# schwallergroup/matinvent

Hardware: AMD Instinct MI355X
Metric: crystal structures/sec (1000-step reverse diffusion) (higher is better)
Workload: dtype f32 via 2-plane fp16 split (3 fp16 MFMA terms, f32 accumulate)

## Files before the change

matinvent_amd/csrc/backward.hip:

```cpp
#include "gemm_split.h"
#include "net.h"

namespace mi {
extern int g_edge_pairs;
int g_tn_xsilu = 1;
int g_bwd_pairs_tile = 1;
int g_bwd_pairs_fused = 1;
int g_bwd_dz2_planes = 1;
int g_bwd_wgrad_planes = 1;
int g_bwd_head_window = 1;
int g_bwd_wgrad_f16 = 1;
}

namespace mi {

__global__ void transpose_kernel(const float* __restrict__ src, int ld_src, int rows, int cols, float* __restrict__ dst) {
    int idx = blockIdx.x * blockDim.x + threadIdx.x;
    if (idx >= rows * cols) return;
    int c = idx / rows, r = idx % rows;
    dst[idx] = src[(size_t)r * ld_src + c];
}

__global__ void silu_bwd_kernel(const float* __restrict__ dy, const float* __restrict__ z, float* __restrict__ out, int64_t n) {
    int64_t i = (int64_t)blockIdx.x * blockDim.x + threadIdx.x;
// ... 1221 lines not shown
    const float s2 = sigma * sigma;
#pragma unroll
    for (int i = -10; i <= 10; ++i) {
        float v = x + (float)i;
        float e = expf(-(v * v) / 2.0f / s2);
        num += v / s2 * e;
        den += e;
    }
    return num / den;
}

struct NoiseArgs {
    const float *lengths, *angles, *frac0;
    const int* atom_types;
    const float *rand_l, *rand_x, *rand_t;
    const int* node_off;
    float *in_lat, *in_frac, *in_types, *tar_x;
    float *out_rand_l, *out_rand_t;
    float c0, c1, sigma, sigma_norm;
    uint64_t seed;
    uint32_t step;
    int64_t node_offset, graph_offset;
    int stack_B0 = 0, stack_N0 = 0;
    float sc0[MI_MAX_STACK], sc1[MI_MAX_STACK], ssig[MI_MAX_STACK], ssn[MI_MAX_STACK];
    const float* sched = nullptr;
};

__global__ __launch_bounds__(256) void add_noise_kernel(NoiseArgs a) {
    const int b = blockIdx.x, tid = threadIdx.x;
    const int cp = a.stack_B0 ? b / a.stack_B0 : 0;
    const float c0 = a.sched ? a.sched[b * 4] : a.stack_B0 ? a.sc0[cp] : a.c0, c1 = a.sched ? a.sched[b * 4 + 1] : a.stack_B0 ? a.sc1[cp] : a.c1;
    const float sigma = a.sched ? a.sched[b * 4 + 2] : a.stack_B0 ? a.ssig[cp] : a.sigma;
    const float sigma_norm = a.sched ? a.sched[b * 4 + 3] : a.stack_B0 ? a.ssn[cp] : a.sigma_norm;
    const uint32_t step = a.step + (uint32_t)cp;
    const int64_t gsub = (int64_t)cp * a.stack_B0, nsub = (int64_t)cp * a.stack_N0;
    __shared__ float Lm[9];
    if (tid == 0) lattice_matrix(a.lengths + b * 3, a.angles + b * 3, Lm);
    __syncthreads();
    if (tid < 9) {
        int idx = b * 9 + tid;
        float z = a.rand_l ? a.rand_l[idx] : philox_normal1(a.seed, step, DRAW_FT_L, (uint64_t)(a.graph_offset - gsub) * 9 + idx);
        a.out_rand_l[idx] = z;
        a.in_lat[idx] = c0 * Lm[tid] + c1 * z;
    }
    const int n0 = a.node_off[b], n1 = a.node_off[b + 1];
    for (int idx = n0 * 3 + tid; idx < n1 * 3; idx += 256) {
        float z = a.rand_x ? a.rand_x[idx] : philox_normal1(a.seed, step, DRAW_FT_X, (uint64_t)(a.node_offset - nsub) * 3 + idx);
        float sx = sigma * z;
        a.in_frac[idx] = pymod1(a.frac0[idx] + sx);
        a.tar_x[idx] = d_log_p_wn(sx, sigma) / sqrtf(sigma_norm);
    }
    for (int64_t idx = (int64_t)n0 * MI_NUM_TYPES + tid; idx < (int64_t)n1 * MI_NUM_TYPES; idx += 256) {
        int i = (int)(idx / MI_NUM_TYPES), k = (int)(idx % MI_NUM_TYPES);
        float z = a.rand_t ? a.rand_t[idx] : philox_normal1(a.seed, step, DRAW_FT_T, (uint64_t)(a.node_offset - nsub) * MI_NUM_TYPES + idx);
        float onehot = (a.atom_types[i] - 1 == k) ? 1.f : 0.f;
        a.out_rand_t[idx] = z;
        a.in_types[idx] = c0 * onehot + c1 * z;
    }
}

struct StackTimes {
    int t[MI_MAX_STACK];
};
__global__ void fill_stack_times_kernel(int* __restrict__ times, StackTimes st, int B0, int B) {
    int b = blockIdx.x * blockDim.x + threadIdx.x;
    if (b < B) times[b] = st.t[b / B0];
}


}

using namespace mi;

extern "C" {

int mi_cspnet_forward_train(mi_net* net, mi_batch* b, const float* t_emb, const float* atom_types, const float* frac,
                            const float* lattices, float* lattice_out, float* coord_out, float* type_out, void* stream) {
    MI_POOL_STREAM(b, stream, "mi_cspnet_forward_train");
    MI_CHECK(net && b, MI_EINVAL, "null handle");
    MI_CHECK(b->H == net->H && b->L == net->L, MI_EINVAL, "batch was created for a different network");
    MI_TRY(net_tape_prepare(net, b));
    return net_forward(net, b, t_emb, atom_types, frac, lattices, lattice_out, coord_out, type_out, (hipStream_t)stream, true);
}

int mi_cspnet_backward(mi_net* net, mi_batch* b, const float* d_lattice_out, const float* d_coord_out, const float* d_type_out,
                       float* grad_theta, void* stream) {
    MI_POOL_STREAM(b, stream, "mi_cspnet_backward");
    MI_CHECK(net && b && d_lattice_out && d_coord_out && d_type_out && grad_theta, MI_EINVAL, "null argument");
    MI_CHECK(net->W2T != nullptr, MI_ESTATE, "mi_net_set_params must run before backward");
    return net_backward(net, b, d_lattice_out, d_coord_out, d_type_out, grad_theta, (hipStream_t)stream);
}

int mi_batch_set_wgrad_window(mi_net* net, mi_batch* b, int micro_steps) {
    MI_CHECK(net && b, MI_EINVAL, "null handle");
    MI_CHECK(b->H == net->H && b->L == net->L, MI_EINVAL, "batch was created for a different network");
    return net_wgrad_window(net, b, micro_steps);
}

int mi_cspnet_wgrad_flush(mi_net* net, mi_batch* b, float* grad_theta, void* stream) {
    MI_POOL_STREAM(b, stream, "mi_cspnet_wgrad_flush");
    MI_CHECK(net && b && grad_theta, MI_EINVAL, "null argument");
    return net_wgrad_flush(net, b, grad_theta, (hipStream_t)stream);
}

int mi_batch_wgrad_pending(const mi_batch* b) { return b ? b->tape.wcur : 0; }

int mi_adam_step(float* theta, const float* grad, float* exp_avg, float* exp_avg_sq, int64_t n, int step, float lr, float beta1,
                 float beta2, float eps, float grad_scale, void* stream) {
    MI_CHECK(theta && grad && exp_avg && exp_avg_sq && n >= 0 && step >= 1, MI_EINVAL, "bad argument");
    if (n == 0) return MI_OK;
    const double bc1 = 1.0 - pow((double)beta1, step), bc2 = 1.0 - pow((double)beta2, step);
    hipLaunchKernelGGL(adam_kernel, dim3((unsigned)cdiv(n, 256)), dim3(256), 0, (hipStream_t)stream, theta, grad, exp_avg, exp_avg_sq, n,
                       (float)(lr / bc1), (float)(1.0 / sqrt(bc2)), beta1, beta2, eps, grad_scale);
    MI_KERNEL_CHECK();
    return MI_OK;
}

int mi_add_noise(mi_batch* b, const float* lengths, const float* angles, const float* frac0, const int* atom_types, float c0, float c1,
                 float sigma, float sigma_norm, uint64_t seed, uint32_t step, const float* rand_l, const float* rand_x, const float* rand_t,
                 float* in_lattice, float* in_frac, float* in_types, float* tar_x, float* out_rand_l, float* out_rand_t, void* stream) {
    MI_NO_POOLED(b, "mi_add_noise");
    MI_CHECK(b && lengths && angles && frac0 && atom_types && in_lattice && in_frac && in_types && tar_x && out_rand_l && out_rand_t,
             MI_EINVAL, "null argument");
    if (b->B == 0) return MI_OK;
    NoiseArgs a{lengths, angles, frac0, atom_types, rand_l, rand_x, rand_t, b->node_off, in_lattice, in_frac, in_types, tar_x,
                out_rand_l, out_rand_t, c0, c1, sigma, sigma_norm, seed, step, b->node_offset, b->graph_offset};
    hipLaunchKernelGGL(add_noise_kernel, dim3(b->B), dim3(256), 0, (hipStream_t)stream, a);
    MI_KERNEL_CHECK();
    return MI_OK;
}

int mi_add_noise_per_crystal(mi_batch* b, const float* lengths, const float* angles, const float* frac0, const int* atom_types,
                             const float* sched, uint64_t seed, uint32_t step, const float* rand_l, const float* rand_x, const float* rand_t,
                             float* in_lattice, float* in_frac, float* in_types, float* tar_x, float* out_rand_l, float* out_rand_t,
                             void* stream) {
    MI_CHECK(b && lengths && angles && frac0 && atom_types && sched && in_lattice && in_frac && in_types && tar_x && out_rand_l && out_rand_t,
             MI_EINVAL, "null argument");
    if (b->B == 0) return MI_OK;
    NoiseArgs a{lengths, angles, frac0, atom_types, rand_l, rand_x, rand_t, b->node_off, in_lattice, in_frac, in_types, tar_x,
                out_rand_l, out_rand_t, 0.f, 0.f, 0.f, 0.f, seed, step, b->node_offset, b->graph_offset};
    a.sched = sched;
    hipLaunchKernelGGL(add_noise_kernel, dim3(b->B), dim3(256), 0, (hipStream_t)stream, a);
    MI_KERNEL_CHECK();
    return MI_OK;
}

}

namespace mi {

int ft_micro_run(const char* what, mi_net* agent, mi_batch* ab, mi_net* prior, mi_batch* pb, const float* lengths, const float* angles,
                 const float* frac0, const int* atom_types, const float* time_freqs, int t, float c0, float c1, float sigma_t, float sigma_norm,
                 int copies, const int* ts, const float* c0s, const float* c1s, const float* sigmas, const float* sigma_norms, uint64_t seed,
                 uint32_t noise_step, const float* rand_l, const float* rand_x, const float* rand_t, float cost_lattice, float cost_coord,
                 float cost_type, int accum_steps, float* grad_theta, ft_loss_stage_fn stage, void* stage_ctx, void* stream, void* aux_stream) {
    MI_CHECK(agent && ab && prior && pb && lengths && angles && frac0 && atom_types && time_freqs && grad_theta && stage, MI_EINVAL,
             "null argument");
    TraceRange range(what);
    MI_CHECK(ab != pb, MI_EINVAL, "agent and prior need separate batch handles (separate workspace)");
    MI_CHECK(ab->B == pb->B && ab->N == pb->N && accum_steps >= 1, MI_EINVAL, "inconsistent batch arguments");
    hipStream_t s = (hipStream_t)stream;
    const int B = ab->B, N = ab->N;
    if (B == 0 || N == 0) return MI_OK;
    MI_TRY(net_tape_prepare(agent, ab));
    Tape& tp = ab->tape;
    const bool hw = tp.head_window();
    const size_t hs = hw ? (size_t)tp.wcur : 0;
    float* const nz_types = hw ? tp.w_types + hs * N * MI_NUM_TYPES : tp.nz_types;
    float* const temb = hw ? tp.w_temb + hs * B * agent->TD : ab->temb;
    float* const d_t = hw ? tp.w_dtype + hs * N * MI_NUM_TYPES : tp.d_t;
    float* const d_x = hw ? tp.w_dcoord + hs * N * 3 : tp.d_x;
    NoiseArgs na{lengths, angles, frac0, atom_types, rand_l, rand_x, rand_t, ab->node_off, tp.nz_lat, tp.nz_frac, nz_types, tp.tar_x,
                 tp.rnd_l, tp.rnd_t, c0, c1, sigma_t, sigma_norm, seed, noise_step, ab->node_offset, ab->graph_offset};
    if (copies > 0) {
        MI_CHECK(copies <= MI_MAX_STACK && B % copies == 0 && N % copies == 0 && ts && c0s && c1s && sigmas && sigma_norms, MI_EINVAL,
                 "stacked micro-step: %d replicas do not fit the batch (B = %d, N = %d) or the limit %d", copies, B, N, MI_MAX_STACK);
        StackTimes st;
        na.stack_B0 = B / copies;
        na.stack_N0 = N / copies;
        for (int c = 0; c < copies; ++c) {
            st.t[c] = ts[c];
            na.sc0[c] = c0s[c];
            na.sc1[c] = c1s[c];
            na.ssig[c] = sigmas[c];
            na.ssn[c] = sigma_norms[c];
        }
        hipLaunchKernelGGL(fill_stack_times_kernel, dim3(cdiv(B, 256)), dim3(256), 0, s, ab->times, st, na.stack_B0, B);
    } else {
        hipLaunchKernelGGL(fill_int_kernel2, dim3(cdiv(B, 256)), dim3(256), 0, s, ab->times, t, B);
    }
    MI_TRY(mi_time_embedding(ab->times, time_freqs, B, agent->TD, temb, stream));
    hipLaunchKernelGGL(add_noise_kernel, dim3(B), dim3(256), 0, s, na);
    MI_KERNEL_CHECK();
    if (aux_stream && aux_stream != stream) {
        hipStream_t s2 = (hipStream_t)aux_stream;
        if (!pb->ev_fork) {
            MI_HIP(hipEventCreateWithFlags(&pb->ev_fork, hipEventDisableTiming));
            MI_HIP(hipEventCreateWithFlags(&pb->ev_join, hipEventDisableTiming));
        }
        MI_HIP(hipEventRecord(pb->ev_fork, s));
        MI_HIP(hipStreamWaitEvent(s2, pb->ev_fork, 0));
        MI_TRY(net_forward(prior, pb, temb, nz_types, tp.nz_frac, tp.nz_lat, pb->pred_l, pb->pred_x, pb->pred_t, s2, false));
        MI_HIP(hipEventRecord(pb->ev_join, s2));
        tp.borrow_inputs = true;
        const int rc = net_forward(agent, ab, temb, nz_types, tp.nz_frac, tp.nz_lat, ab->pred_l, ab->pred_x, ab->pred_t, s, true);
        tp.borrow_inputs = false;
        MI_TRY(rc);
        MI_HIP(hipStreamWaitEvent(s, pb->ev_join, 0));
    } else {
        tp.borrow_inputs = true;
        const int rc = net_forward(agent, ab, temb, nz_types, tp.nz_frac, tp.nz_lat, ab->pred_l, ab->pred_x, ab->pred_t, s, true);
        tp.borrow_inputs = false;
        MI_TRY(rc);
        MI_TRY(net_forward(prior, pb, temb, nz_types, tp.nz_frac, tp.nz_lat, pb->pred_l, pb->pred_x, pb->pred_t, s, false));
    }
    FtStageIO io{ab->pred_l, ab->pred_x, ab->pred_t, pb->pred_l, pb->pred_x, pb->pred_t, tp.rnd_l, tp.tar_x, tp.rnd_t, ab->node_off,
                 tp.d_l, d_x, d_t, tp.Lb, tp.KLb, B, N, cost_lattice, cost_coord, cost_type, accum_steps};
    MI_TRY(stage(io, stage_ctx, s));
    return net_backward(agent, ab, tp.d_l, d_x, d_t, grad_theta, s);
}

}

struct FtRewardStage {
    const float* reward;
    float kl_sigma;
    int b_global;
    float *stats, *out_sample_loss, *out_kl;
};
static int ft_reward_stage(const FtStageIO& io, void* ctx, hipStream_t s) {
    const FtRewardStage& c = *(const FtRewardStage*)ctx;
    const int B = io.B;
    LossArgs la{io.pl, io.px, io.pt, io.plp, io.pxp, io.ptp, io.rl, io.tx, io.rt, c.reward, io.node_off,
                io.dl, io.dx, io.dt, io.Lb, io.KLb, io.cl, io.cx, io.ct, c.kl_sigma,
                1.0f / ((float)c.b_global * (float)io.accum_steps)};
    hipLaunchKernelGGL(ft_loss_kernel, dim3(B), dim3(256), 0, s, la);
    if (c.stats) hipLaunchKernelGGL(ft_stats_kernel, dim3(1), dim3(64), 0, s, io.Lb, io.KLb, c.reward, B, c.kl_sigma, 1.0f / (float)c.b_global, c.stats);
    MI_KERNEL_CHECK();
    if (c.out_sample_loss) MI_HIP(hipMemcpyAsync(c.out_sample_loss, io.Lb, B * 4, hipMemcpyDeviceToDevice, s));
    if (c.out_kl) MI_HIP(hipMemcpyAsync(c.out_kl, io.KLb, B * 4, hipMemcpyDeviceToDevice, s));
    return MI_OK;
}

static int ft_micro_impl(mi_net* agent, mi_batch* ab, mi_net* prior, mi_batch* pb, const float* lengths, const float* angles,
                         const float* frac0, const int* atom_types, const float* reward, const float* time_freqs, int t, float c0, float c1,
                         float sigma_t, float sigma_norm, int copies, const int* ts, const float* c0s, const float* c1s, const float* sigmas,
                         const float* sigma_norms, uint64_t seed, uint32_t noise_step, const float* rand_l, const float* rand_x,
                         const float* rand_t, float cost_lattice, float cost_coord, float cost_type, float kl_sigma, int b_global,
                         int accum_steps, float* grad_theta, float* stats, float* out_sample_loss, float* out_kl, void* stream,
                         void* aux_stream) {
    MI_CHECK(reward, MI_EINVAL, "null argument");
    MI_CHECK(!ab || b_global >= ab->B / (copies > 0 ? copies : 1), MI_EINVAL, "inconsistent batch arguments");
    FtRewardStage st{reward, kl_sigma, b_global, stats, out_sample_loss, out_kl};
    return ft_micro_run("mi_ft_micro_step", agent, ab, prior, pb, lengths, angles, frac0, atom_types, time_freqs, t, c0, c1, sigma_t, sigma_norm,
                        copies, ts, c0s, c1s, sigmas, sigma_norms, seed, noise_step, rand_l, rand_x, rand_t, cost_lattice, cost_coord, cost_type,
                        accum_steps, grad_theta, ft_reward_stage, &st, stream, aux_stream);
}

extern "C" {

int mi_ft_micro_step(mi_net* agent, mi_batch* ab, mi_net* prior, mi_batch* pb, const float* lengths, const float* angles,
                     const float* frac0, const int* atom_types, const float* reward, const float* time_freqs, int t, float c0, float c1,
                     float sigma_t, float sigma_norm, uint64_t seed, uint32_t noise_step, const float* rand_l, const float* rand_x,
                     const float* rand_t, float cost_lattice, float cost_coord, float cost_type, float kl_sigma, int b_global, int accum_steps,
                     float* grad_theta, float* stats, float* out_sample_loss, float* out_kl, void* stream, void* aux_stream) {
    MI_NO_LATENT(agent, "mi_ft_micro_step");
    MI_NO_LATENT(prior, "mi_ft_micro_step");
    MI_NO_POOLED(ab, "mi_ft_micro_step");
    MI_NO_POOLED(pb, "mi_ft_micro_step");
    return ft_micro_impl(agent, ab, prior, pb, lengths, angles, frac0, atom_types, reward, time_freqs, t, c0, c1, sigma_t, sigma_norm, 0, nullptr,
                         nullptr, nullptr, nullptr, nullptr, seed, noise_step, rand_l, rand_x, rand_t, cost_lattice, cost_coord, cost_type,
                         kl_sigma, b_global, accum_steps, grad_theta, stats, out_sample_loss, out_kl, stream, aux_stream);
}

int mi_ft_micro_steps_stacked(mi_net* agent, mi_batch* ab, mi_net* prior, mi_batch* pb, const float* lengths, const float* angles,
                              const float* frac0, const int* atom_types, const float* reward, const float* time_freqs, int copies,
                              const int* t_host, const float* c0_host, const float* c1_host, const float* sigma_t_host,
                              const float* sigma_norm_host, uint64_t seed, uint32_t noise_step, const float* rand_l, const float* rand_x,
                              const float* rand_t, float cost_lattice, float cost_coord, float cost_type, float kl_sigma, int b_global,
                              int accum_steps, float* grad_theta, float* stats, void* stream, void* aux_stream) {
    MI_NO_LATENT(agent, "mi_ft_micro_steps_stacked");
    MI_NO_LATENT(prior, "mi_ft_micro_steps_stacked");
    MI_NO_POOLED(ab, "mi_ft_micro_steps_stacked");
    MI_NO_POOLED(pb, "mi_ft_micro_steps_stacked");
    MI_CHECK(copies >= 1, MI_EINVAL, "copies must be positive");
    return ft_micro_impl(agent, ab, prior, pb, lengths, angles, frac0, atom_types, reward, time_freqs, 0, 0.f, 0.f, 0.f, 0.f, copies, t_host,
                         c0_host, c1_host, sigma_t_host, sigma_norm_host, seed, noise_step, rand_l, rand_x, rand_t, cost_lattice, cost_coord,
                         cost_type, kl_sigma, b_global, accum_steps, grad_theta, stats, nullptr, nullptr, stream, aux_stream);
}

int mi_debug_gemm(int kind, const float* A, int lda, const float* W, int ldw, float* C, int ldc, int M, int N, int K, void* stream) {
    MI_CHECK(A && W && C, MI_EINVAL, "null argument");
    if (kind == 2 || kind == 3) {
        static u16 *pa = nullptr, *pw = nullptr;
        static size_t na = 0, nw = 0;
        hipStream_t s = (hipStream_t)stream;
        if (planes_elems(M, K) > na) { if (pa) (void)hipFree(pa); na = planes_elems(M, K); MI_HIP(hipMalloc((void**)&pa, na * 2)); }
        if (planes_elems(N, K) > nw) { if (pw) (void)hipFree(pw); nw = planes_elems(N, K); MI_HIP(hipMalloc((void**)&pw, nw * 2)); }
        Planes PA = make_planes(pa, K, PL_S_LN), PW = make_planes(pw, K, PL_SW);
        if (ldc >= 0) {
            hipLaunchKernelGGL(split_planes_kernel<>, dim3(cdiv((int64_t)((M + 127) / 128 * 128) * PA.KT * 16, 256)), dim3(256), 0, s, A, lda, M, K, PA);
            hipLaunchKernelGGL(split_planes_kernel<>, dim3(cdiv((int64_t)((N + 127) / 128 * 128) * PW.KT * 16, 256)), dim3(256), 0, s, W, ldw, N, K, PW);
        }
        if (MI_PLANES_FP16 && (N & 255) == 0 && (K & 63) == 0 && K >= 128) {
            static u16* pf = nullptr;
            static size_t nf = 0;
            if (frag_elems(N, K) > nf) { if (pf) (void)hipFree(pf); nf = frag_elems(N, K); MI_HIP(hipMalloc((void**)&pf, nf * 2)); }
            MI_TRY(pack_frag_from_planes(PW, N, K, pf, s));
            PW.frag = pf;
        }
        PlanesEpilogue pe;
        pe.C = C;
        pe.ldc = ldc < 0 ? -ldc : ldc;
        const int saved = g_planes_variant;
        g_planes_variant = kind == 3;
        const int rc = gemm_planes(PA, PW, M, N, K, pe, s);
        g_planes_variant = saved;
        return rc;
    }
#if MI_PLANES_FP16
    if (kind == 5) {
        hipStream_t s = (hipStream_t)stream;
        MI_CHECK(M % 256 == 0 && N % 128 == 0 && K >= 4096, MI_EINVAL, "kind 5: the plane-set weight-gradient form needs M % 256 == 0, N % 128 == 0, K >= 4096");
        static u16 *pa = nullptr, *pw = nullptr;
        static float *sc = nullptr, *dsc = nullptr;
        static size_t na = 0, nw = 0;
        const size_t ea = planes_elems(K, M), ew = planes_elems(K, N), scf = (size_t)1 << 25;
        if (ea > na) { if (pa) (void)hipFree(pa); na = ea; MI_HIP(hipMalloc((void**)&pa, na * 2)); }
        if (ew > nw) { if (pw) (void)hipFree(pw); nw = ew; MI_HIP(hipMalloc((void**)&pw, nw * 2)); }
        if (!sc) MI_HIP(hipMalloc((void**)&sc, scf * sizeof(float)));
        if (!dsc) {
            MI_HIP(hipMalloc((void**)&dsc, 2 * sizeof(float)));
            const float h[2] = {64.f, 1.f / 64.f};
            MI_HIP(hipMemcpy(dsc, h, sizeof(h), hipMemcpyHostToDevice));
        }
        Planes PA = make_planes(pa, M, 64.f), PW = make_planes(pw, N, 64.f);
        hipLaunchKernelGGL(split_planes_kernel<>, dim3(cdiv((int64_t)((K + 127) / 128 * 128) * PA.KT * 16, 256)), dim3(256), 0, s, A, lda, K, M, PA);
        hipLaunchKernelGGL(split_planes_kernel<>, dim3(cdiv((int64_t)((K + 127) / 128 * 128) * PW.KT * 16, 256)), dim3(256), 0, s, W, ldw, K, N, PW);
        MI_KERNEL_CHECK();
        MI_CHECK(gemm_tn_planes_ok(PA, 0, PW, 0, K, M, N), MI_EINVAL, "kind 5: shape outside the plane-set form");
        return gemm_tn_planes(PA, 0, PW, 0, C, ldc, K, M, N, dsc, dsc, sc, scf, s);
    }
#endif
    if (kind == 4) {
        static float* sc = nullptr;
        const size_t scf = (size_t)1 << 24;
        if (!sc) MI_HIP(hipMalloc((void**)&sc, scf * sizeof(float)));
        return gemm_tn_auto(A, lda, W, ldw, C, ldc, K, M, N, sc, scf, (hipStream_t)stream);
    }
    return kind == 0 ? gemm_nt_f32(A, lda, W, ldw, C, ldc, M, N, K, GemmEpilogue(), (hipStream_t)stream)
                     : gemm_nt_split(A, lda, W, ldw, C, ldc, M, N, K, GemmEpilogue(), (hipStream_t)stream);
}

}
```

matinvent_amd/csrc/edge_stage.hip:

```cpp
#include <mutex>

#include <cstdio>
#include <cstdlib>
#include "net.h"
#include "gemm_split.h"
#define MI_LOOP_BARRIER() __builtin_amdgcn_s_barrier()
#define MI_RING_WAIT(w) asm volatile("s_waitcnt vmcnt(20)" : "+v"((w)[0][0]), "+v"((w)[0][1]), "+v"((w)[1][0]), "+v"((w)[1][1]))

namespace mi {

extern int g_edge2_train;
int g_edge2_fused = 1;

#if MI_PLANES_FP16

struct EdgeGemm2Args {
    Planes A;
    const u16* W2f;
    const float* b2;
    const float* dsc;
    const int* src;
    const int* rowptr;
    float* part;
    int E, N;
    const int* tab = nullptr;
    float* Z2 = nullptr;
    unsigned long long* clk;
};

constexpr int EG2_TAB = 2 + 128 + 128;
__global__ __launch_bounds__(128) void edge2_tables_kernel(const int* __restrict__ src, const int* __restrict__ rowptr, int E, int N, int* __restrict__ tab) {
    const int tile = blockIdx.x, tid = threadIdx.x, row0 = tile * 128;
    if (row0 >= E) return;
    const int nrows = E - row0 < 128 ? E - row0 : 128;
    const int node_first = src[row0];
    int* t = tab + (size_t)tile * EG2_TAB;
    const int r = row0 + tid, node = node_first + tid;
    t[2 + tid] = r < E ? src[r] - node_first : -1;
    t[130 + tid] = node < N ? tile - (rowptr[node] >> 7) : 0;
    if (tid == 0) {
        t[0] = node_first;
        t[1] = src[row0 + nrows - 1] - node_first + 1;
    }
}

constexpr int EG2B_STAGE = 2 * 128 * 64, EG2B_NST = 4;
constexpr int EG2B_LDS = EG2B_NST * EG2B_STAGE + 128 * 4 + 128 * 4;

template <int D, bool SAVE_Z = false>
__global__ __launch_bounds__(256) __attribute__((amdgpu_waves_per_eu(2, 2))) void edge_gemm2b_kernel(EdgeGemm2Args a) {
    constexpr int H = 512, KS = H / 16, KT = H / 32;
    extern __shared__ __attribute__((aligned(16))) unsigned char smem[];
    int* srcl = reinterpret_cast<int*>(smem + EG2B_NST * EG2B_STAGE);
    int* slotb = srcl + 128;
    const int tid = threadIdx.x, lane = tid & 63, wave = __builtin_amdgcn_readfirstlane(tid >> 6);
    const int l31 = lane & 31, kg = lane >> 5;
    const int id = blockIdx.x, slot = id >> 3, half = slot & 1, tile = (slot >> 1) * 8 + (id & 7);
    const int row0 = tile * 128;
    if (row0 >= a.E) return;
    const int nrows = a.E - row0 < 128 ? a.E - row0 : 128;
    int stamp_i = 0;
    auto stamp = [&]() {
        if (a.clk && tid == 0) a.clk[(size_t)(tile * 2 + half) * 8 + stamp_i] = __builtin_amdgcn_s_memtime();
        ++stamp_i;
    };
    stamp();
    if (a.clk && tid == 0) a.clk[(size_t)(tile * 2 + half) * 8 + 4] = __builtin_amdgcn_s_memrealtime();

    const int* tab = a.tab + (size_t)tile * EG2_TAB;
    int t_srcl = -1, t_slotb = 0;
    if (tid < 128) {
        t_srcl = tab[2 + tid];
        t_slotb = tab[130 + tid];
    }
    const int node_first = tab[0], cnt_tab = tab[1];

    const __amdgpu_buffer_rsrc_t rsa = uniform_rsrc(a.A.base + a.A.tile(tile, 0), a.A.KT * 24576);
    const int voffa = (lane >> 2) * 64 + (((lane & 3) ^ ((lane >> 4) & 3)) << 4);
    auto dma_tile = [&](int kt, int st) {
#pragma unroll
        for (int q = 0; q < 4; ++q) {
            const int piece = wave * 4 + q;
            __builtin_amdgcn_raw_ptr_buffer_load_lds(rsa, (__attribute__((address_space(3))) void*)(smem + st * EG2B_STAGE + piece * 1024), 16, voffa,
                                                     kt * 24576 + (piece >> 3) * 8192 + (piece & 7) * 1024, 0, 0);
        }
    };
    dma_tile(0, 0);
    dma_tile(1, 1);
    dma_tile(2, 2);

    int voffw[2];
#pragma unroll
    for (int t = 0; t < 2; ++t) voffw[t] = lane * 16 + ((8 * half + 2 * wave + t) * KS) * 2048;
    u32x4 ring[D][2][2];
    const u32x4 rsw_s = rsrc_words(a.W2f, H * H * 4);
    auto ring_load = [&](int ks, u32x4 (&w)[2][2]) {
        const int soff = __builtin_amdgcn_readfirstlane(ks * 2048);
#pragma unroll
        for (int t = 0; t < 2; ++t) {
            asm volatile("buffer_load_dwordx4 %0, %1, %2, %3 offen" : "=v"(w[t][0]) : "v"(voffw[t]), "s"(rsw_s), "s"(soff));
            asm volatile("buffer_load_dwordx4 %0, %1, %2, %3 offen offset:1024" : "=v"(w[t][1]) : "v"(voffw[t]), "s"(rsw_s), "s"(soff));
        }
    };
#pragma unroll
    for (int d = 0; d < D; ++d) ring_load(d, ring[d]);

    if (tid < 128) {
        srcl[tid] = t_srcl;
        slotb[tid] = t_slotb;
    }
    const float os = a.dsc[1] * (1.f / PL_SW), s_m2 = a.dsc[2], inv_m2 = a.dsc[3];

    f32x16 acc[4][2];
#pragma unroll
    for (int i = 0; i < 4; ++i)
#pragma unroll
        for (int j = 0; j < 2; ++j)
#pragma unroll
            for (int r = 0; r < 16; ++r) acc[i][j][r] = 0.f;
    const unsigned lds0 = (unsigned)(uintptr_t)(__attribute__((address_space(3))) unsigned char*)smem;
    unsigned rd_off[2];
#pragma unroll
    for (int s2 = 0; s2 < 2; ++s2) rd_off[s2] = lds0 + (unsigned)(l31 * 64 + (((2 * s2 + kg) ^ ((l31 >> 2) & 3)) * 16));
    auto read_a = [&](int st, int s2, f16x8 (&af)[4][2]) {
        const unsigned va = rd_off[s2] + (unsigned)st * EG2B_STAGE;
#define MI_RD128(dst, off) asm volatile("ds_read_b128 %0, %1 offset:%2" : "=v"(dst) : "v"(va), "n"(off))
        MI_RD128(af[0][0], 0 * 2048);        MI_RD128(af[0][1], 0 * 2048 + 8192);
        MI_RD128(af[1][0], 1 * 2048);        MI_RD128(af[1][1], 1 * 2048 + 8192);
        MI_RD128(af[2][0], 2 * 2048);        MI_RD128(af[2][1], 2 * 2048 + 8192);
        MI_RD128(af[3][0], 3 * 2048);        MI_RD128(af[3][1], 3 * 2048 + 8192);
#undef MI_RD128
    };
    auto mma = [&](const u32x4 (&w)[2][2], f16x8 (&af)[4][2]) {
#pragma unroll
        for (int ip = 0; ip < 2; ++ip) {
            if (ip == 0) asm volatile("s_waitcnt lgkmcnt(4)" : "+v"(af[0][0]), "+v"(af[0][1]), "+v"(af[1][0]), "+v"(af[1][1]));
            else asm volatile("s_waitcnt lgkmcnt(0)" : "+v"(af[2][0]), "+v"(af[2][1]), "+v"(af[3][0]), "+v"(af[3][1]));
#pragma unroll
            for (int term = MI_TERM0; term < 3; ++term)
#pragma unroll
                for (int i = 2 * ip; i < 2 * ip + 2; ++i)
#pragma unroll
                    for (int j = 0; j < 2; ++j)
                        acc[i][j] = __builtin_amdgcn_mfma_f32_32x32x16_f16(af[i][term == 0 ? 1 : 0], __builtin_bit_cast(f16x8, w[j][term == 1 ? 1 : 0]), acc[i][j], 0, 0, 0);
        }
    };
    static_assert(D == 4, "two k-tiles of ring per unrolled pair of iterations");
#pragma unroll 1
    for (int kt = 0; kt < KT; kt += 2) {
#pragma unroll
        for (int h2 = 0; h2 < 2; ++h2) {
            const int k = kt + h2;
            if (k == 0 || k >= KT - 3) asm volatile("s_waitcnt vmcnt(0)" ::: "memory");
            else asm volatile("s_waitcnt vmcnt(24)" ::: "memory");
            MI_LOOP_BARRIER();
            if (k == 0) stamp();
            if (k + 3 < KT) dma_tile(k + 3, (k + 3) & 3);
            f16x8 af[4][2];
#pragma unroll
            for (int s2 = 0; s2 < 2; ++s2) {
                read_a(k & 3, s2, af);
                MI_RING_WAIT(ring[2 * h2 + s2]);
                mma(ring[2 * h2 + s2], af);
                if (2 * k + s2 + D < KS) ring_load(2 * k + s2 + D, ring[2 * h2 + s2]);
                __builtin_amdgcn_sched_barrier(0);
            }
        }
    }
    stamp();

    if constexpr (SAVE_Z) {
        __syncthreads();
        float* stage = reinterpret_cast<float*>(smem) + wave * 1152;
#pragma unroll
        for (int i = 0; i < 4; ++i)
#pragma unroll
            for (int j = 0; j < 2; ++j) {
                const int rb = row0 + i * 32, cb = half * 256 + wave * 64 + j * 32;
#pragma unroll
                for (int r = 0; r < 16; ++r) stage[((r & 3) + 8 * (r >> 2) + 4 * kg) * 36 + l31] = acc[i][j][r] * os;
                __builtin_amdgcn_wave_barrier();
#pragma unroll
                for (int u = 0; u < 2; ++u) {
                    const int q = lane + 64 * u, rl = q >> 2, c8 = (q & 3) * 8;
                    const int row = rb + rl, col = cb + c8;
                    f32x4 z0 = *reinterpret_cast<const f32x4*>(stage + rl * 36 + c8);
                    f32x4 z1 = *reinterpret_cast<const f32x4*>(stage + rl * 36 + c8 + 4);
                    if (row < a.E) {
                        z0 += *reinterpret_cast<const f32x4*>(a.b2 + col);
                        z1 += *reinterpret_cast<const f32x4*>(a.b2 + col + 4);
                        float* d = a.Z2 + (size_t)row * H + col;
                        *reinterpret_cast<f32x4*>(d) = z0;
                        *reinterpret_cast<f32x4*>(d + 4) = z1;
                    }
                }
                __builtin_amdgcn_wave_barrier();
            }
    }

    const int cnt = nrows > 0 ? cnt_tab : 0;
    u16* sfr = reinterpret_cast<u16*>(smem);
    unsigned sat = 0;
    const int nlb = (cnt + 31) >> 5;
    __syncthreads();
    for (int f = tid; f < nlb * 8 * 64; f += 256) {
        const int ln = f & 63, fu = (f >> 6) & 1, frb = (f >> 7) & 3, fq = f >> 9;
        const int me = fq * 32 + (ln & 31), fkg = ln >> 5;
        u32x4 w;
#pragma unroll
        for (int i2 = 0; i2 < 4; ++i2) {
            const int ia = 2 * i2, ib = 2 * i2 + 1;
            const int ra = frb * 32 + 4 * fkg + 8 * (2 * fu + (ia >> 2)) + (ia & 3), rbb = frb * 32 + 4 * fkg + 8 * (2 * fu + (ib >> 2)) + (ib & 3);
            w[i2] = (srcl[ra] == me ? 0x3C00u : 0u) | (srcl[rbb] == me ? 0x3C000000u : 0u);
        }
        *reinterpret_cast<u32x4*>(sfr + (size_t)f * 8) = w;
    }
    __syncthreads();
#pragma unroll
    for (int j = 0; j < 2; ++j) {
        __builtin_amdgcn_sched_barrier(0);
        const int col = half * 256 + wave * 64 + j * 32 + l31;
        const float bcol = a.b2[col];
#pragma unroll 1
        for (int lb0 = 0; lb0 < nlb; lb0 += 2) {
            const bool two = lb0 + 1 < nlb;
            f32x16 ps[2];
#pragma unroll
            for (int q = 0; q < 2; ++q)
#pragma unroll
                for (int r = 0; r < 16; ++r) ps[q][r] = 0.f;
#pragma unroll
            for (int rb = 0; rb < 4; ++rb) {
                const f32x16 av = acc[rb][j];
#pragma unroll
                for (int u = 0; u < 2; ++u) {
                    f16x8 mh, ml;
#pragma unroll
                    for (int idx = 0; idx < 8; idx += 2) {
                        const float v0 = silu_fast(av[8 * u + idx] * os + bcol), v1 = silu_fast(av[8 * u + idx + 1] * os + bcol);
                        unsigned p[3];
                        pl_split_pair_acc(v0, v1, s_m2, p, sat);
                        const f16x2 h = __builtin_bit_cast(f16x2, p[0]), lo = __builtin_bit_cast(f16x2, p[1]);
                        mh[idx] = h[0]; mh[idx + 1] = h[1];
                        ml[idx] = lo[0]; ml[idx + 1] = lo[1];
                    }
#pragma unroll
                    for (int q = 0; q < 2; ++q) {
                        if (q == 1 && !two) break;
                        const f16x8 sf = *reinterpret_cast<const f16x8*>(sfr + (size_t)((((lb0 + q) * 4 + rb) * 2 + u) * 64 + lane) * 8);
                        ps[q] = __builtin_amdgcn_mfma_f32_32x32x16_f16(sf, ml, ps[q], 0, 0, 0);
                        ps[q] = __builtin_amdgcn_mfma_f32_32x32x16_f16(sf, mh, ps[q], 0, 0, 0);
                    }
                    __builtin_amdgcn_sched_barrier(0);
                }
            }
#pragma unroll
            for (int q = 0; q < 2; ++q)
#pragma unroll
                for (int r = 0; r < 16; ++r) {
                    const int loc = (lb0 + q) * 32 + (r & 3) + 8 * (r >> 2) + 4 * kg;
                    if (loc < cnt) a.part[((size_t)slotb[loc] * a.N + node_first + loc) * H + col] = ps[q][r] * inv_m2;
                }
        }
    }
    stamp();
    if (a.clk && tid == 0) a.clk[(size_t)(tile * 2 + half) * 8 + 5] = __builtin_amdgcn_s_memrealtime();
    sat_report(sat);
}

template <bool EXT, bool LEAN = false>
__global__ __launch_bounds__(256) __attribute__((amdgpu_waves_per_eu(2, 2))) void gemm_rt_kernel(Planes A, const u16* __restrict__ Wf, int M, int N, int K,
                                                                                                 PlanesEpilogue pe, unsigned long long* __restrict__ clk) {
    const int KS = K >> 4, KT = K >> 5;
    extern __shared__ __attribute__((aligned(16))) unsigned char smem[];
    M = pe.rows(M);
    const int tid = threadIdx.x, lane = tid & 63, wave = __builtin_amdgcn_readfirstlane(tid >> 6);
    int stamp_i = 0;
    auto stamp = [&]() {
        if (clk && tid == 0) clk[(size_t)blockIdx.x * 8 + stamp_i] = __builtin_amdgcn_s_memtime();
        ++stamp_i;
    };
    stamp();
    if (clk && tid == 0) clk[(size_t)blockIdx.x * 8 + 4] = __builtin_amdgcn_s_memrealtime();
    const int l31 = lane & 31, kg = lane >> 5;
    const int ncb = N >> 8;
    const int id = blockIdx.x, slot = id >> 3, cb = slot % ncb, tile = (slot / ncb) * 8 + (id & 7);
    const int row0 = tile * 128;
    if (row0 >= M) return;

    const __amdgpu_buffer_rsrc_t rsa = uniform_rsrc(A.base + A.tile(tile, 0), A.KT * 24576);
    const int voffa = (lane >> 2) * 64 + (((lane & 3) ^ ((lane >> 4) & 3)) << 4);
    auto dma_tile = [&](int kt, int st) {
#pragma unroll
        for (int q = 0; q < 4; ++q) {
            const int piece = wave * 4 + q;
            __builtin_amdgcn_raw_ptr_buffer_load_lds(rsa, (__attribute__((address_space(3))) void*)(smem + st * EG2B_STAGE + piece * 1024), 16, voffa,
                                                     kt * 24576 + (piece >> 3) * 8192 + (piece & 7) * 1024, 0, 0);
        }
    };
    dma_tile(0, 0);
    dma_tile(1, 1);
    dma_tile(2, 2);

    int voffw[2];
#pragma unroll
    for (int t = 0; t < 2; ++t) voffw[t] = lane * 16 + ((8 * cb + 2 * wave + t) * KS) * 2048;
    u32x4 ring[4][2][2];
    const u32x4 rsw_s = rsrc_words(Wf, N * K * 4);
    auto ring_load = [&](int ks, u32x4 (&w)[2][2]) {
        const int soff = __builtin_amdgcn_readfirstlane(ks * 2048);
#pragma unroll
        for (int t = 0; t < 2; ++t) {
            asm volatile("buffer_load_dwordx4 %0, %1, %2, %3 offen" : "=v"(w[t][0]) : "v"(voffw[t]), "s"(rsw_s), "s"(soff));
            asm volatile("buffer_load_dwordx4 %0, %1, %2, %3 offen offset:1024" : "=v"(w[t][1]) : "v"(voffw[t]), "s"(rsw_s), "s"(soff));
        }
    };
#pragma unroll
    for (int d = 0; d < 4; ++d) ring_load(d, ring[d]);

    f32x16 acc[4][2];
#pragma unroll
    for (int i = 0; i < 4; ++i)
#pragma unroll
        for (int j = 0; j < 2; ++j)
#pragma unroll
            for (int r = 0; r < 16; ++r) acc[i][j][r] = 0.f;
    const unsigned lds0 = (unsigned)(uintptr_t)(__attribute__((address_space(3))) unsigned char*)smem;
    unsigned rd_off[2];
#pragma unroll
    for (int s2 = 0; s2 < 2; ++s2) rd_off[s2] = lds0 + (unsigned)(l31 * 64 + (((2 * s2 + kg) ^ ((l31 >> 2) & 3)) * 16));
    auto read_a = [&](int st, int s2, f16x8 (&af)[4][2]) {
        const unsigned va = rd_off[s2] + (unsigned)st * EG2B_STAGE;
#define MI_RD128(dst, off) asm volatile("ds_read_b128 %0, %1 offset:%2" : "=v"(dst) : "v"(va), "n"(off))
        MI_RD128(af[0][0], 0 * 2048);        MI_RD128(af[0][1], 0 * 2048 + 8192);
        MI_RD128(af[1][0], 1 * 2048);        MI_RD128(af[1][1], 1 * 2048 + 8192);
        MI_RD128(af[2][0], 2 * 2048);        MI_RD128(af[2][1], 2 * 2048 + 8192);
        MI_RD128(af[3][0], 3 * 2048);        MI_RD128(af[3][1], 3 * 2048 + 8192);
#undef MI_RD128
    };
    auto mma = [&](const u32x4 (&w)[2][2], f16x8 (&af)[4][2]) {
#pragma unroll
        for (int ip = 0; ip < 2; ++ip) {
            if (ip == 0) asm volatile("s_waitcnt lgkmcnt(4)" : "+v"(af[0][0]), "+v"(af[0][1]), "+v"(af[1][0]), "+v"(af[1][1]));
            else asm volatile("s_waitcnt lgkmcnt(0)" : "+v"(af[2][0]), "+v"(af[2][1]), "+v"(af[3][0]), "+v"(af[3][1]));
#pragma unroll
            for (int term = MI_TERM0; term < 3; ++term)
#pragma unroll
                for (int i = 2 * ip; i < 2 * ip + 2; ++i)
#pragma unroll
                    for (int j = 0; j < 2; ++j)
                        if constexpr (LEAN)
                            acc[i][j] = __builtin_amdgcn_mfma_f32_32x32x16_f16(__builtin_bit_cast(f16x8, w[j][term == 1 ? 1 : 0]), af[i][term == 0 ? 1 : 0], acc[i][j], 0, 0, 0);
                        else
                            acc[i][j] = __builtin_amdgcn_mfma_f32_32x32x16_f16(af[i][term == 0 ? 1 : 0], __builtin_bit_cast(f16x8, w[j][term == 1 ? 1 : 0]), acc[i][j], 0, 0, 0);
        }
    };
#pragma unroll 1
    for (int kt = 0; kt < KT; kt += 2) {
#pragma unroll
        for (int h2 = 0; h2 < 2; ++h2) {
            const int k = kt + h2;
            if (k == 0 || k >= KT - 3) asm volatile("s_waitcnt vmcnt(0)" ::: "memory");
            else asm volatile("s_waitcnt vmcnt(24)" ::: "memory");
            MI_LOOP_BARRIER();
            if (k == 0) stamp();
            if (k + 3 < KT) dma_tile(k + 3, (k + 3) & 3);
            f16x8 af[4][2];
#pragma unroll
            for (int s2 = 0; s2 < 2; ++s2) {
                read_a(k & 3, s2, af);
                MI_RING_WAIT(ring[2 * h2 + s2]);
                mma(ring[2 * h2 + s2], af);
                if (2 * k + s2 + 4 < KS) ring_load(2 * k + s2 + 4, ring[2 * h2 + s2]);
                __builtin_amdgcn_sched_barrier(0);
            }
        }
    }
    __syncthreads();
    stamp();
    if constexpr (LEAN) planes_epilogue_lean<4, 2>(pe, acc, tile, cb * 256 + wave * 64, M, lane);
    else planes_epilogue_rows<4, 2, EXT>(pe, acc, row0, cb * 256 + wave * 64, M, N, lane, reinterpret_cast<float*>(smem) + wave * 1152);
    stamp();
    if (clk && tid == 0) clk[(size_t)blockIdx.x * 8 + 5] = __builtin_amdgcn_s_memrealtime();
}

__global__ void pack_frag_from_planes_kernel(Planes W, int N, int K, u16* __restrict__ dst) {
    const int KS = K / 16;
    const int64_t idx = (int64_t)blockIdx.x * blockDim.x + threadIdx.x;
    if (idx >= (int64_t)N * (K / 8)) return;
    const int r = (int)(idx / (K / 8)), ch = (int)(idx % (K / 8));
    const int ct = r >> 5, l31 = r & 31, ks = ch >> 1, kg = ch & 1;
#pragma unroll
    for (int pl = 0; pl < 2; ++pl)
        *reinterpret_cast<u32x4*>(dst + ((((size_t)ct * KS + ks) * 2 + pl) * 64 + kg * 32 + l31) * 8) = *reinterpret_cast<const u32x4*>(W.base + W.elem(r, ch * 8, pl));
}

int g_edge1_fused = 9;

__global__ void pack_frag_wff_pair_kernel(const float* __restrict__ W1, int edge_in, int H, int F, int Kh, u16* __restrict__ dst) {
    const int K = 2 * Kh, KS = K / 16, F3 = 3 * F;
    const int64_t idx = (int64_t)blockIdx.x * blockDim.x + threadIdx.x;
    if (idx >= (int64_t)H * (K / 8)) return;
    const int r = (int)(idx / (K / 8)), ch = (int)(idx % (K / 8));
    const int ct = r >> 5, l31 = r & 31, ks = ch >> 1, kg = ch & 1;
    float v[8];
#pragma unroll
    for (int i = 0; i < 8; ++i) {
        const int c = ch * 8 + i, blk = c >= Kh, cc = blk ? c - Kh : c;
        v[i] = cc < F3 ? W1[(size_t)r * edge_in + 2 * H + 9 + blk * F3 + cc] : 0.f;
    }
    u32x4 pk[2];
#pragma unroll
    for (int i = 0; i < 4; ++i) {
        unsigned p[3];
        pl_split_pair(v[2 * i], v[2 * i + 1], PL_SW, p);
        pk[0][i] = p[0];
        pk[1][i] = p[1];
    }
#pragma unroll
    for (int pl = 0; pl < 2; ++pl) *reinterpret_cast<u32x4*>(dst + ((((size_t)ct * KS + ks) * 2 + pl) * 64 + kg * 32 + l31) * 8) = pk[pl];
}

template <int D, bool WIDE>
__device__ __forceinline__ void edge_gemm1_body(const Planes& A, const u16* __restrict__ Wf, int M, int N, int K, PlanesEpilogue& pe, unsigned long long* clk) {
    extern __shared__ __attribute__((aligned(16))) unsigned char smem[];
    const int tid = threadIdx.x, lane = tid & 63, wave = __builtin_amdgcn_readfirstlane(tid >> 6);
    const int l31 = lane & 31, kg = lane >> 5;
    constexpr int MI = 4, NJ = 1;
    constexpr int WM = 4 / MI, WN = 4 / WM, WGC = 32 * NJ * WN;
    const int KT = K / 32, KS = K / 16, nq = N / WGC;
    const int wm = wave / WN, wn = wave % WN;
    const int id = blockIdx.x;
    float cps_local = 0.f;
    auto eval_scales = [&]() {
        if (pe.sc_pq) {
            float dsc[6];
            act_scales_eval(__uint_as_float(pe.sc_pq[0]), __uint_as_float(pe.sc_gmax[0]), pe.sc_wb, dsc);
            cps_local = dsc[0];
            if (id == 0 && tid < 6) {
                pe.sc_dsc[tid] = dsc[tid];
                if (pe.sc_dsc2) pe.sc_dsc2[tid] = dsc[tid];
            }
        }
    };
    eval_scales();
    if (pe.diag_C0 && id >= pe.diag_block0) {
        const float cps = cps_local != 0.f ? cps_local : pe.Cp.s();
        const int n0 = (id - pe.diag_block0) * 8, n1 = n0 + 8 < pe.diag_nodes ? n0 + 8 : pe.diag_nodes;
        const float* PQ = pe.ep.row_bias;
        const int ldpq = pe.ep.ld_row_bias;
        for (int f = 2 * tid; f < N; f += 512) {
            const float c0 = pe.diag_C0[f], c1 = pe.diag_C0[f + 1];
            for (int i = n0; i < n1; ++i) {
                const int e = pe.diag_e[i], g = pe.diag_node2graph[i];
                const float* G = pe.ep.row_bias3 + (size_t)g * pe.ep.ld_row_bias3;
                const float v0 = c0 + ((PQ[(size_t)i * ldpq + f] + PQ[(size_t)i * ldpq + N + f]) + G[f]);
                const float v1 = c1 + ((PQ[(size_t)i * ldpq + f + 1] + PQ[(size_t)i * ldpq + N + f + 1]) + G[f + 1]);
                if (pe.ep.pre_act) {
                    pe.ep.pre_act[(size_t)e * pe.ep.ld_pre + f] = v0;
                    pe.ep.pre_act[(size_t)e * pe.ep.ld_pre + f + 1] = v1;
                }
                unsigned p[3];
                pl_split_pair(silu_fast(v0), silu_fast(v1), cps, p);
#pragma unroll
                for (int k = 0; k < NPL; ++k) *reinterpret_cast<unsigned*>(pe.Cp.base + pe.Cp.elem(e, f, k)) = p[k];
            }
        }
        return;
    }
    const int slot = id >> 3, qt = slot % nq, tile = (slot / nq) * 8 + (id & 7);
    const int row0 = tile * 128;
    if (row0 >= M) return;
    int stamp_i = 0;
    auto stamp = [&]() {
        if (clk && tid == 0) clk[(size_t)(tile * nq + qt) * 8 + stamp_i] = __builtin_amdgcn_s_memtime();
        ++stamp_i;
    };
    stamp();

    const __amdgpu_buffer_rsrc_t rsa = uniform_rsrc(A.base + A.tile(tile, 0), A.KT * 24576);
    const int voffa = (lane >> 2) * 64 + (((lane & 3) ^ ((lane >> 4) & 3)) << 4);
    auto dma_tile = [&](int kt, int st) {
#pragma unroll
        for (int q = 0; q < 4; ++q) {
            const int piece = wave * 4 + q;
            __builtin_amdgcn_raw_ptr_buffer_load_lds(rsa, (__attribute__((address_space(3))) void*)(smem + st * EG2B_STAGE + piece * 1024), 16, voffa,
                                                     kt * 24576 + (piece >> 3) * 8192 + (piece & 7) * 1024, 0, 0);
        }
    };
    dma_tile(0, 0);
    dma_tile(1, 1);
    dma_tile(2, 2);
    const __amdgpu_buffer_rsrc_t rsw = uniform_rsrc(Wf, N * K * 4);
    int voffw[NJ];
#pragma unroll
    for (int t = 0; t < NJ; ++t) voffw[t] = lane * 16 + (((WN * qt + wn) * NJ + t) * KS) * 2048;
    u32x4 ring[D][NJ][2];
    const u32x4 rsw_s = rsrc_words(Wf, N * K * 4);
    auto ring_load = [&](int ks, u32x4 (&w)[NJ][2]) {
        const int soff = __builtin_amdgcn_readfirstlane(ks * 2048);
        asm volatile("buffer_load_dwordx4 %0, %1, %2, %3 offen" : "=v"(w[0][0]) : "v"(voffw[0]), "s"(rsw_s), "s"(soff));
        asm volatile("buffer_load_dwordx4 %0, %1, %2, %3 offen offset:1024" : "=v"(w[0][1]) : "v"(voffw[0]), "s"(rsw_s), "s"(soff));
    };
#pragma unroll
    for (int d = 0; d < D; ++d) ring_load(d, ring[d]);

    f32x16 acc[MI][NJ], accS[MI][NJ];
#pragma unroll
    for (int i = 0; i < MI; ++i)
#pragma unroll
        for (int j = 0; j < NJ; ++j)
#pragma unroll
            for (int r = 0; r < 16; ++r) acc[i][j][r] = 0.f;
    const unsigned lds0 = (unsigned)(uintptr_t)(__attribute__((address_space(3))) unsigned char*)smem;
    unsigned rd_off[2];
#pragma unroll
    for (int s2 = 0; s2 < 2; ++s2) rd_off[s2] = lds0 + (unsigned)(l31 * 64 + (((2 * s2 + kg) ^ ((l31 >> 2) & 3)) * 16));
    auto read_a = [&](int st, int s2, f16x8 (&af)[MI][2]) {
        const unsigned va = rd_off[s2] + (unsigned)st * EG2B_STAGE;
#define MI_RD128(dst, off) asm volatile("ds_read_b128 %0, %1 offset:%2" : "=v"(dst) : "v"(va), "n"(off))
        MI_RD128(af[0][0], 0 * 2048);        MI_RD128(af[0][1], 0 * 2048 + 8192);
        MI_RD128(af[1][0], 1 * 2048);        MI_RD128(af[1][1], 1 * 2048 + 8192);
        MI_RD128(af[2][0], 2 * 2048);        MI_RD128(af[2][1], 2 * 2048 + 8192);
        MI_RD128(af[3][0], 3 * 2048);        MI_RD128(af[3][1], 3 * 2048 + 8192);
#undef MI_RD128
    };
    auto mma = [&](u32x4 (&w)[NJ][2], f16x8 (&af)[MI][2]) {
        asm volatile("s_waitcnt vmcnt(14)" : "+v"(w[0][0]), "+v"(w[0][1]));
#pragma unroll
        for (int ip = 0; ip < 2; ++ip) {
            if (ip == 0) asm volatile("s_waitcnt lgkmcnt(4)" : "+v"(af[0][0]), "+v"(af[0][1]), "+v"(af[1][0]), "+v"(af[1][1]));
            else asm volatile("s_waitcnt lgkmcnt(0)" : "+v"(af[2][0]), "+v"(af[2][1]), "+v"(af[3][0]), "+v"(af[3][1]));
#pragma unroll
            for (int term = MI_TERM0; term < 3; ++term)
#pragma unroll
                for (int i = 2 * ip; i < 2 * ip + 2; ++i)
                    acc[i][0] = __builtin_amdgcn_mfma_f32_32x32x16_f16(af[i][term == 0 ? 1 : 0], __builtin_bit_cast(f16x8, w[0][term == 1 ? 1 : 0]), acc[i][0], 0, 0, 0);
        }
    };
    static_assert(D == 4, "two k-tiles of ring per unrolled pair of iterations");
    const int khalf = KT / 2;
#pragma unroll 1
    for (int kt = 0; kt < KT; kt += 2) {
#pragma unroll
        for (int h2 = 0; h2 < 2; ++h2) {
            const int k = kt + h2;
            if (k == khalf) {
#pragma unroll
                for (int i = 0; i < MI; ++i)
#pragma unroll
                    for (int j = 0; j < NJ; ++j) {
                        accS[i][j] = acc[i][j];
#pragma unroll
                        for (int r = 0; r < 16; ++r) acc[i][j][r] = 0.f;
                    }
            }
            if (k == 0 || k >= KT - 3) asm volatile("s_waitcnt vmcnt(0)" ::: "memory");
            else asm volatile("s_waitcnt vmcnt(16)" ::: "memory");
            MI_LOOP_BARRIER();
            if (k == 0) stamp();
            if (k + 3 < KT) dma_tile(k + 3, (k + 3) & 3);
            f16x8 af[MI][2];
#pragma unroll
            for (int s2 = 0; s2 < 2; ++s2) {
                read_a(k & 3, s2, af);
                mma(ring[2 * h2 + s2], af);
                if (2 * k + s2 + D < KS) ring_load(2 * k + s2 + D, ring[2 * h2 + s2]);
                __builtin_amdgcn_sched_barrier(0);
            }
        }
    }
    stamp();
    __syncthreads();
    planes_epilogue_pairs<MI, NJ, WIDE>(pe, accS, acc, row0 + wm * MI * 32, qt * WGC + wn * 32 * NJ, M, N, lane, reinterpret_cast<float*>(smem) + wave * 2304, cps_local);
    stamp();
}

template <int D, bool WIDE = true>
__global__ __launch_bounds__(256) __attribute__((amdgpu_waves_per_eu(2, 2))) void edge_gemm1b_kernel(Planes A, const u16* __restrict__ Wf, int M, int N, int K,
                                                                                                     PlanesEpilogue pe, unsigned long long* clk) {
    edge_gemm1_body<D, WIDE>(A, Wf, M, N, K, pe, clk);
}

unsigned long long* g_edge1_clk = nullptr;

__global__ void empty_boundary_kernel() {}

int edge_gemm1(mi_net* net, const Planes& A, int layer, int M, PlanesEpilogue pe, hipStream_t s) {
    if (g_ablate_skip & 2) return MI_OK;
    if (g_ablate_skip & 32) hipLaunchKernelGGL(empty_boundary_kernel, dim3(1), dim3(64), 0, s);
    static std::once_flag once;
    static hipError_t attr_err = hipSuccess;
    std::call_once(once, [] {
        attr_err = hipFuncSetAttribute((const void*)edge_gemm1b_kernel<4>, hipFuncAttributeMaxDynamicSharedMemorySize, EG2B_LDS);
        if (attr_err == hipSuccess) attr_err = hipFuncSetAttribute((const void*)edge_gemm1b_kernel<4, false>, hipFuncAttributeMaxDynamicSharedMemorySize, EG2B_LDS);
    });
    MI_HIP(attr_err);
    const int H = net->H, K = 2 * net->Kh;
    count_mfma(M, H, K, MI_PLANES_TERMS);
    pe.out_scale = 1.f / (A.scale * PL_SW);
    int nblk = (H / 128) * ((cdiv(M, 128) + 7) / 8 * 8);
    if (pe.diag_C0) {
        pe.diag_block0 = nblk;
        nblk += cdiv(pe.diag_nodes, 8);
    }
    const u16* Wf = net->Wffc + (size_t)layer * ((size_t)H * K * 2);
    if (pe.pair_wide) hipLaunchKernelGGL((edge_gemm1b_kernel<4>), dim3(nblk), dim3(256), EG2B_LDS, s, A, Wf, M, H, K, pe, g_edge1_clk);
    else hipLaunchKernelGGL((edge_gemm1b_kernel<4, false>), dim3(nblk), dim3(256), EG2B_LDS, s, A, Wf, M, H, K, pe, g_edge1_clk);
    MI_KERNEL_CHECK();
    return MI_OK;
}

bool edge_gemm1_supported(const mi_net* net, int64_t M) {
    if (!(net->H % 128 == 0 && net->Wffc != nullptr && (2 * net->Kh) % 64 == 0) || g_edge1_fused == 0) return false;
    if (g_edge1_fused != 9) return true;
    return (int64_t)(net->H / 128) * ((cdiv(M, 128) + 7) / 8 * 8) > g_planes_lat_max_blocks;
}

int edge_gemm1_pack(mi_net* net, int l, const float* W1, hipStream_t s) {
    const int H = net->H, K = 2 * net->Kh;
    hipLaunchKernelGGL(pack_frag_wff_pair_kernel, dim3(cdiv((int64_t)H * (K / 8), 256)), dim3(256), 0, s, W1, net->edge_in, H, net->F, net->Kh,
                       net->Wffc + (size_t)l * ((size_t)H * K * 2));
    MI_KERNEL_CHECK();
    return MI_OK;
}

unsigned long long* g_edge2_clk = nullptr;

int edge_gemm2(mi_net* net, mi_batch* b, int layer, hipStream_t s, float* Z2) {
    if (g_ablate_skip & 4) return MI_OK;
    if (g_ablate_skip & 32) hipLaunchKernelGGL(empty_boundary_kernel, dim3(1), dim3(64), 0, s);
    static std::once_flag once;
    static hipError_t attr_err = hipSuccess;
    std::call_once(once, [] {
        attr_err = hipFuncSetAttribute((const void*)edge_gemm2b_kernel<4>, hipFuncAttributeMaxDynamicSharedMemorySize, EG2B_LDS);
        if (attr_err == hipSuccess) attr_err = hipFuncSetAttribute((const void*)edge_gemm2b_kernel<4, true>, hipFuncAttributeMaxDynamicSharedMemorySize, EG2B_LDS);
    });
    MI_HIP(attr_err);
    const int H = net->H;
    count_mfma(b->E, H, H, MI_PLANES_TERMS);
    EdgeGemm2Args a;
    a.A = make_planes(b->m1_cur ? b->m1_cur : b->M1pl, H, PL_S_ACT, b->dsc);
    a.W2f = net->Wnc + (size_t)layer * node_chain_pack_elems(H) + (size_t)5 * H * H * 2;
    a.b2 = net->p("csp_layer_" + std::to_string(layer) + ".edge_mlp.2.bias");
    a.dsc = b->dsc;
    a.src = b->src;
    a.rowptr = b->rowptr;
    a.part = b->part;
    a.E = (int)b->E;
    a.N = b->N;
    {
        const int tiles_cap = cdiv(b->E_cap, 128);
        if (!b->e2_tab) MI_TRY(dev_alloc(b, &b->e2_tab, (size_t)tiles_cap * EG2_TAB));
        if (b->e2_tab_epoch != b->graph_epoch) {
            hipLaunchKernelGGL(edge2_tables_kernel, dim3(cdiv(b->E, 128)), dim3(128), 0, s, b->src, b->rowptr, (int)b->E, b->N, b->e2_tab);
            MI_KERNEL_CHECK();
            b->e2_tab_epoch = b->graph_epoch;
        }
        a.tab = b->e2_tab;
    }
    a.Z2 = Z2;
    a.clk = g_edge2_clk;
    if (Z2) {
        hipLaunchKernelGGL((edge_gemm2b_kernel<4, true>), dim3(2 * ((cdiv(b->E, 128) + 7) / 8 * 8)), dim3(256), EG2B_LDS, s, a);
        MI_KERNEL_CHECK();
        return MI_OK;
    }
    hipLaunchKernelGGL((edge_gemm2b_kernel<4>), dim3(2 * ((cdiv(b->E, 128) + 7) / 8 * 8)), dim3(256), EG2B_LDS, s, a);
    MI_KERNEL_CHECK();
    return MI_OK;
}

bool edge_gemm2_supported(const mi_net* net) { return g_edge2_fused && net->H == 512 && net->Wnc != nullptr; }

unsigned long long* g_rt_clk = nullptr;
int g_rt_clk_ext = -1;
int g_rt_lean = 1;
int g_rt_clk_skip = 0;

int gemm_rt(const Planes& A, const u16* Wfrag, int M, int N, int K, const PlanesEpilogue& pe, bool ext, hipStream_t s) {
    static std::once_flag once;
    static hipError_t attr_err = hipSuccess;
    std::call_once(once, [] {
        attr_err = hipFuncSetAttribute((const void*)gemm_rt_kernel<false>, hipFuncAttributeMaxDynamicSharedMemorySize, EG2B_NST * EG2B_STAGE);
        if (attr_err == hipSuccess) attr_err = hipFuncSetAttribute((const void*)gemm_rt_kernel<true>, hipFuncAttributeMaxDynamicSharedMemorySize, EG2B_NST * EG2B_STAGE);
        if (attr_err == hipSuccess) attr_err = hipFuncSetAttribute((const void*)gemm_rt_kernel<false, true>, hipFuncAttributeMaxDynamicSharedMemorySize, EG2B_NST * EG2B_STAGE);
        if (const char* e = getenv("MI_RT_LEAN")) g_rt_lean = atoi(e) & 3;
    });
    MI_HIP(attr_err);
    MI_CHECK(Wfrag && (N & 255) == 0 && (K & 63) == 0 && K >= 128 && A.KT >= K / 32, MI_EINVAL, "gemm_rt: N % 256, K % 64, K >= 128 and a fragment-order W operand");
    if (M <= 0) return MI_OK;
    count_mfma(M, N, K, MI_PLANES_TERMS);
    const dim3 grid((N >> 8) * ((cdiv(M, 128) + 7) / 8 * 8));
    static const bool trace = getenv("MI_RT_TRACE") != nullptr;
    if (trace)
        fprintf(stderr, "gemm_rt M=%d N=%d K=%d ext=%d act=%d bias=%d rb=%d%d%d pre_add=%d pre_act=%d res=%d res_pl=%d os=%g res2=%d res2_pl=%d rows2=%d post_mul=%d C=%d Cp=%d absmax=%d\n", M, N, K,
                (int)ext, pe.ep.act, !!pe.ep.bias, !!pe.ep.row_bias, !!pe.ep.row_bias2, !!pe.ep.row_bias3, !!pe.ep.pre_add, !!pe.ep.pre_act, !!pe.ep.residual, !!pe.res_pl.base,
                (double)pe.ep.out_scale, !!pe.residual2, !!pe.res2_pl.base, !!pe.res2_rows, !!pe.post_mul, !!pe.C, !!pe.Cp.base, !!pe.absmax);
    unsigned long long* clk = nullptr;
    if (g_rt_clk && (g_rt_clk_ext < 0 || g_rt_clk_ext == (int)ext)) {
        if (g_rt_clk_skip > 0) {
            --g_rt_clk_skip;
        } else {
            clk = g_rt_clk;
            if (g_rt_clk_ext >= 0) g_rt_clk = nullptr;
        }
    }
    if (g_rt_lean && planes_epilogue_is_lean(pe)) hipLaunchKernelGGL((gemm_rt_kernel<false, true>), grid, dim3(256), EG2B_NST * EG2B_STAGE, s, A, Wfrag, M, N, K, pe, clk);
    else if (ext) hipLaunchKernelGGL(gemm_rt_kernel<true>, grid, dim3(256), EG2B_NST * EG2B_STAGE, s, A, Wfrag, M, N, K, pe, clk);
    else hipLaunchKernelGGL(gemm_rt_kernel<false>, grid, dim3(256), EG2B_NST * EG2B_STAGE, s, A, Wfrag, M, N, K, pe, clk);
    MI_KERNEL_CHECK();
    return MI_OK;
}

size_t frag_elems(int N, int K) { return (size_t)N * K * 2; }

int pack_frag_from_planes(const Planes& W, int N, int K, u16* dst, hipStream_t s) {
    MI_CHECK((N & 31) == 0 && (K & 15) == 0, MI_EINVAL, "pack_frag_from_planes: N % 32, K % 16");
    hipLaunchKernelGGL(pack_frag_from_planes_kernel, dim3((unsigned)cdiv((int64_t)N * (K / 8), 256)), dim3(256), 0, s, W, N, K, dst);
    MI_KERNEL_CHECK();
    return MI_OK;
}

#else

int gemm_rt(const Planes&, const u16*, int, int, int, const PlanesEpilogue&, bool, hipStream_t) { return MI_ESTATE; }
size_t frag_elems(int N, int K) { return (size_t)N * K * 2; }
int pack_frag_from_planes(const Planes&, int, int, u16*, hipStream_t) { return MI_ESTATE; }

int edge_gemm2(mi_net*, mi_batch*, int, hipStream_t, float*) { return MI_ESTATE; }
bool edge_gemm2_supported(const mi_net*) { return false; }
int edge_gemm1(mi_net*, const Planes&, int, int, PlanesEpilogue, hipStream_t) { return MI_ESTATE; }
bool edge_gemm1_supported(const mi_net*, int64_t) { return false; }
int edge_gemm1_pack(mi_net*, int, const float*, hipStream_t) { return MI_OK; }
int g_edge1_fused = 0;

#endif

}

extern "C" int mi_debug_set_rt_lean(int on) {
#if MI_PLANES_FP16
    const int was = mi::g_rt_lean;
    mi::g_rt_lean = on & 3;
    return was;
#else
    (void)on;
    return 0;
#endif
}

extern "C" int mi_debug_rt_clock(void* dev_buffer, int ext, int skip) {
#if MI_PLANES_FP16
    mi::g_rt_clk = (unsigned long long*)dev_buffer;
    mi::g_rt_clk_ext = ext;
    mi::g_rt_clk_skip = skip;
#else
    (void)dev_buffer; (void)ext; (void)skip;
#endif
    return MI_OK;
}

extern "C" int mi_debug_edge2_clock(void* dev_buffer) {
#if MI_PLANES_FP16
    mi::g_edge2_clk = (unsigned long long*)dev_buffer;
#endif
    return MI_OK;
}

extern "C" int mi_debug_edge1_clock(void* dev_buffer) {
#if MI_PLANES_FP16
    mi::g_edge1_clk = (unsigned long long*)dev_buffer;
#endif
    return MI_OK;
}

extern "C" int mi_debug_set_edge2_fused(int on) {
    const int was = (mi::g_edge2_fused == 1 && !mi::g_edge2_train) ? 4 : mi::g_edge2_fused;
    mi::g_edge2_fused = on == 4 ? 1 : on;
    mi::g_edge2_train = on == 1;
    return was;
}

extern "C" int mi_debug_set_edge_fused(int) { return 0; }

extern "C" int mi_debug_set_edge1_fused(int on) {
    const int was = mi::g_edge1_fused;
    mi::g_edge1_fused = on;
    return was;
}
```

matinvent_amd/csrc/gemm_split.h:

```cpp
#pragma once
#include <type_traits>
#include "gemm.h"

namespace mi {

typedef short bf16x8 __attribute__((ext_vector_type(8)));
typedef unsigned short u16;
typedef unsigned u32x4 __attribute__((ext_vector_type(4)));

__device__ __forceinline__ u16 f2bf(float x) {
    unsigned u = __float_as_uint(x);
    u += 0x7FFFu + ((u >> 16) & 1u);
    return (u16)(u >> 16);
}
__device__ __forceinline__ float bf2f(u16 h) { return __uint_as_float(((unsigned)h) << 16); }

__device__ __forceinline__ void split3(float x, u16& p0, u16& p1, u16& p2) {
    p0 = f2bf(x);
    float r = x - bf2f(p0);
    p1 = f2bf(r);
    r = r - bf2f(p1);
    p2 = f2bf(r);
}

// ... 144 lines not shown
    for (int o = 32; o > 0; o >>= 1) m = fmaxf(m, __shfl_xor(m, o, 64));
    if ((threadIdx.x & 63) == 0) atomicMax(out + (blockIdx.x & spread_mask), __float_as_uint(m));
}

template <int BM, int BN, bool F16 = false>
__global__ __launch_bounds__(256) void gemm_nt_split_kernel(const float* __restrict__ A, int lda, const float* __restrict__ W, int ldw,
                                                            float* __restrict__ C, int ldc, int M, int N, int K, GemmEpilogue ep, int kchunk,
                                                            float* __restrict__ part, const unsigned* __restrict__ amax_a = nullptr,
                                                            const unsigned* __restrict__ amax_w = nullptr) {
    constexpr int BK = 32, ROWB = 80;
    constexpr int TM = BM / 64, TN = BN / 64;
    extern __shared__ __attribute__((aligned(16))) unsigned char smem[];
    unsigned char* As = smem;
    unsigned char* Ws = smem + 3 * BM * ROWB;

    const int tid = threadIdx.x, lane = tid & 63, wave = tid >> 6;
    const int wm = wave >> 1, wn = wave & 1, l31 = lane & 31, kg = lane >> 5;
    const int row0 = blockIdx.y * BM, col0 = blockIdx.x * BN;
    const int kbeg = blockIdx.z * kchunk, kend = min(K, kbeg + kchunk);

    f32x16 acc[TM][TN];
#pragma unroll
    for (int i = 0; i < TM; ++i)
#pragma unroll
        for (int j = 0; j < TN; ++j)
#pragma unroll
            for (int r = 0; r < 16; ++r) acc[i][j][r] = 0.f;

    constexpr int A_V = BM * BK / 4 / 256, W_V = BN * BK / 4 / 256;
    f32x4 ra[2][A_V], rw[2][W_V];
    auto load_tiles = [&](int k0, f32x4 (&qa)[A_V], f32x4 (&qw)[W_V]) {
#pragma unroll
        for (int v = 0; v < A_V; ++v) {
            int f = tid + v * 256, r = f >> 3, c = (f & 7) * 4, gr = row0 + r, gk = k0 + c;
            f32x4 val = {0.f, 0.f, 0.f, 0.f};
            if (gr < M && gk < kend) val = *reinterpret_cast<const f32x4*>(A + (size_t)gr * lda + gk);
            qa[v] = val;
        }
#pragma unroll
        for (int v = 0; v < W_V; ++v) {
            int f = tid + v * 256, r = f >> 3, c = (f & 7) * 4, gr = col0 + r, gk = k0 + c;
            f32x4 val = {0.f, 0.f, 0.f, 0.f};
            if (gr < N && gk < kend) val = *reinterpret_cast<const f32x4*>(W + (size_t)gr * ldw + gk);
            qw[v] = val;
        }
    };
    float sc_a = 1.f, sc_w = 1.f;
    if (F16) {
        sc_a = f16_scale_from_absmax(*amax_a);
        sc_w = f16_scale_from_absmax(*amax_w);
    }
    auto store_split = [&](unsigned char* base, int rows, const f32x4& val, int f, float sc) {
        int r = f >> 3, c = (f & 7) * 4;
        unsigned lo[3], hi[3];
        if (F16) {
            const float x0 = val[0] * sc, x1 = val[1] * sc, x2 = val[2] * sc, x3 = val[3] * sc;
            const f16x2 h0 = {(_Float16)x0, (_Float16)x1}, h1 = {(_Float16)x2, (_Float16)x3};
            lo[0] = __builtin_bit_cast(unsigned, h0);
            hi[0] = __builtin_bit_cast(unsigned, h1);
            lo[1] = pack_f16(x0 - (float)h0[0], x1 - (float)h0[1]);
            hi[1] = pack_f16(x2 - (float)h1[0], x3 - (float)h1[1]);
        } else {
            split3_pair(val[0], val[1], lo);
            split3_pair(val[2], val[3], hi);
        }
#pragma unroll
        for (int pl = 0; pl < (F16 ? 2 : 3); ++pl) {
            uint2 pk = {lo[pl], hi[pl]};
            *reinterpret_cast<uint2*>(base + ((size_t)pl * rows + r) * ROWB + c * 2) = pk;
        }
    };
    auto step = [&](int k0, f32x4 (&qa)[A_V], f32x4 (&qw)[W_V]) {
#pragma unroll
        for (int v = 0; v < A_V; ++v) store_split(As, BM, qa[v], tid + v * 256, sc_a);
#pragma unroll
        for (int v = 0; v < W_V; ++v) store_split(Ws, BN, qw[v], tid + v * 256, sc_w);
        __syncthreads();
        load_tiles(k0 + 2 * BK, qa, qw);
#pragma unroll
        for (int s = 0; s < BK / 16; ++s) {
            bf16x8 a[TM][3], b[TN][3];
#pragma unroll
            for (int i = 0; i < TM; ++i)
#pragma unroll
                for (int pl = 0; pl < (F16 ? 2 : 3); ++pl)
                    a[i][pl] = *reinterpret_cast<const bf16x8*>(As + ((size_t)pl * BM + (wm * TM + i) * 32 + l31) * ROWB + (16 * s + 8 * kg) * 2);
#pragma unroll
            for (int j = 0; j < TN; ++j)
#pragma unroll
                for (int pl = 0; pl < (F16 ? 2 : 3); ++pl)
                    b[j][pl] = *reinterpret_cast<const bf16x8*>(Ws + ((size_t)pl * BN + (wn * TN + j) * 32 + l31) * ROWB + (16 * s + 8 * kg) * 2);
#pragma unroll
            for (int i = 0; i < TM; ++i)
#pragma unroll
                for (int j = 0; j < TN; ++j) {
                    if (F16) {
#if !MI_TF32_CLASS
                        acc[i][j] = __builtin_amdgcn_mfma_f32_32x32x16_f16(__builtin_bit_cast(f16x8, a[i][1]), __builtin_bit_cast(f16x8, b[j][0]), acc[i][j], 0, 0, 0);
                        acc[i][j] = __builtin_amdgcn_mfma_f32_32x32x16_f16(__builtin_bit_cast(f16x8, a[i][0]), __builtin_bit_cast(f16x8, b[j][1]), acc[i][j], 0, 0, 0);
#endif
                        acc[i][j] = __builtin_amdgcn_mfma_f32_32x32x16_f16(__builtin_bit_cast(f16x8, a[i][0]), __builtin_bit_cast(f16x8, b[j][0]), acc[i][j], 0, 0, 0);
                        continue;
                    }
                    acc[i][j] = __builtin_amdgcn_mfma_f32_32x32x16_bf16(a[i][2], b[j][0], acc[i][j], 0, 0, 0);
                    acc[i][j] = __builtin_amdgcn_mfma_f32_32x32x16_bf16(a[i][0], b[j][2], acc[i][j], 0, 0, 0);
                    acc[i][j] = __builtin_amdgcn_mfma_f32_32x32x16_bf16(a[i][1], b[j][1], acc[i][j], 0, 0, 0);
                    acc[i][j] = __builtin_amdgcn_mfma_f32_32x32x16_bf16(a[i][1], b[j][0], acc[i][j], 0, 0, 0);
                    acc[i][j] = __builtin_amdgcn_mfma_f32_32x32x16_bf16(a[i][0], b[j][1], acc[i][j], 0, 0, 0);
                    acc[i][j] = __builtin_amdgcn_mfma_f32_32x32x16_bf16(a[i][0], b[j][0], acc[i][j], 0, 0, 0);
                }
        }
        __syncthreads();
    };

    load_tiles(kbeg, ra[0], rw[0]);
    load_tiles(kbeg + BK, ra[1], rw[1]);
    for (int k0 = kbeg; k0 < kend; k0 += 2 * BK) {
        step(k0, ra[0], rw[0]);
        step(k0 + BK, ra[1], rw[1]);
    }

#pragma unroll
    for (int i = 0; i < TM; ++i)
#pragma unroll
        for (int j = 0; j < TN; ++j) {
            int col = col0 + (wn * TN + j) * 32 + l31;
            if (col >= N) continue;
            float bcol = ep.bias ? ep.bias[col] : 0.f;
#pragma unroll
            for (int r = 0; r < 16; ++r) {
                int row = row0 + (wm * TM + i) * 32 + (r & 3) + 8 * (r >> 2) + 4 * kg;
                if (row >= M) continue;
                const float av = F16 ? acc[i][j][r] * (1.0f / (sc_a * sc_w)) : acc[i][j][r];
                if (gridDim.z > 1) {
                    part[((size_t)blockIdx.z * M + row) * N + col] = av;
                    continue;
                }
                float v = av + bcol;
                v = apply_epilogue(ep, v, row, col);
                C[(size_t)row * ldc + col] = v;
            }
        }
}

#ifdef MI_GEMM_OWNER
static __global__ void splitk_reduce_kernel(const float* __restrict__ part, int S, int M, int N, float* __restrict__ C, int ldc, GemmEpilogue ep) {
    const int64_t idx = (int64_t)blockIdx.x * blockDim.x + threadIdx.x;
    if (idx >= (int64_t)M * N) return;
    const int row = (int)(idx / N), col = (int)(idx % N);
    float v = 0.f;
    int z = 0;
    const size_t MN = (size_t)M * N;
    for (; z + 4 <= S; z += 4) {
        const float p0 = part[(size_t)z * MN + idx], p1 = part[(size_t)(z + 1) * MN + idx], p2 = part[(size_t)(z + 2) * MN + idx],
                    p3 = part[(size_t)(z + 3) * MN + idx];
        v += p0;
        v += p1;
        v += p2;
        v += p3;
    }
    for (; z < S; ++z) v += part[(size_t)z * MN + idx];
    v += ep.bias ? ep.bias[col] : 0.f;
    C[(size_t)row * ldc + col] = apply_epilogue(ep, v, row, col);
}
#endif

#ifdef MI_GEMM_OWNER
int gemm_nt_split(const float* A, int lda, const float* W, int ldw, float* C, int ldc, int M, int N, int K, const GemmEpilogue& ep,
                         hipStream_t s, const SplitK* sk = nullptr, const unsigned* amax_a = nullptr, const unsigned* amax_w = nullptr) {
    MI_CHECK(K % 4 == 0 && lda % 4 == 0 && ldw % 4 == 0, MI_EINVAL, "gemm_nt_split: K/lda/ldw must be multiples of 4");
    if (M <= 0 || N <= 0) return MI_OK;
    count_mfma(M, N, K, (amax_a && amax_w && (int64_t)cdiv(M, 128) * cdiv(N, 128) >= 256) ? (MI_TF32_CLASS ? 1 : 3) : (MI_TF32_CLASS ? 1 : 6));
    if ((int64_t)cdiv(M, 128) * cdiv(N, 128) >= 256) {
        constexpr int BM = 128, BN = 128;
        if (amax_a && amax_w)
            hipLaunchKernelGGL((gemm_nt_split_kernel<BM, BN, true>), dim3(cdiv(N, BN), cdiv(M, BM)), dim3(256), 3 * (BM + BN) * 80, s, A, lda, W, ldw, C,
                               ldc, M, N, K, ep, K, (float*)nullptr, amax_a, amax_w);
        else
            hipLaunchKernelGGL((gemm_nt_split_kernel<BM, BN>), dim3(cdiv(N, BN), cdiv(M, BM)), dim3(256), 3 * (BM + BN) * 80, s, A, lda, W, ldw, C, ldc,
                               M, N, K, ep, K, (float*)nullptr, (const unsigned*)nullptr, (const unsigned*)nullptr);
    } else {
        constexpr int BM = 64, BN = 64;
        const int tiles = cdiv(M, BM) * cdiv(N, BN);
        int S = 1;
        if (sk && sk->buf && tiles <= 128 && K >= 256) {
            S = std::min(8, K / 128);
            while (S > 1 && (tiles * S > 512 || (size_t)S * M * N > sk->floats)) --S;
        }
        const int kchunk = S > 1 ? cdiv(cdiv(K, S), 64) * 64 : K;
        S = cdiv(K, kchunk);
        hipLaunchKernelGGL((gemm_nt_split_kernel<BM, BN>), dim3(cdiv(N, BN), cdiv(M, BM), S), dim3(256), 3 * (BM + BN) * 80, s, A, lda, W, ldw, C,
                           ldc, M, N, K, ep, kchunk, S > 1 ? sk->buf : (float*)nullptr, (const unsigned*)nullptr, (const unsigned*)nullptr);
        if (S > 1) hipLaunchKernelGGL(splitk_reduce_kernel, dim3(cdiv((int64_t)M * N, 256)), dim3(256), 0, s, sk->buf, S, M, N, C, ldc, ep);
    }
    MI_KERNEL_CHECK();
    return MI_OK;
}
#else
int gemm_nt_split(const float* A, int lda, const float* W, int ldw, float* C, int ldc, int M, int N, int K, const GemmEpilogue& ep,
                         hipStream_t s, const SplitK* sk = nullptr, const unsigned* amax_a = nullptr, const unsigned* amax_w = nullptr);
#endif

extern int g_gemm_mode;
extern int g_planes_variant;
extern int g_planes_db_min_tiles;
extern int g_planes_small_tiles;
extern int g_planes_big;
extern int g_planes_big_min_rows;
extern int g_planes_rt;
extern int g_planes_rt_min_rows;
extern int g_planes_dma;
extern int g_planes_lat_max_blocks;
extern int g_pair_kernel;
inline int gemm_nt(const float* A, int lda, const float* W, int ldw, float* C, int ldc, int M, int N, int K, const GemmEpilogue& ep,
                   hipStream_t s, const SplitK* sk = nullptr) {
    return g_gemm_mode == 0 ? gemm_nt_f32(A, lda, W, ldw, C, ldc, M, N, K, ep, s) : gemm_nt_split(A, lda, W, ldw, C, ldc, M, N, K, ep, s, sk);
}

}

namespace mi {

struct Planes {
    u16* base = nullptr;
    int KT = 0;
    float scale = 1.f;
    const float* dscale = nullptr;
    const u16* frag = nullptr;
    __device__ __forceinline__ float s() const { return dscale ? dscale[0] : scale; }
    __host__ __device__ size_t tile(int rt, int kt) const { return (size_t)rt * ((size_t)KT * 12288 + 2048) + (size_t)kt * 12288; }
    __host__ __device__ size_t elem(int r, int c, int p) const { return tile(r >> 7, c >> 5) + (size_t)p * 4096 + (r & 127) * 32 + (c & 31); }
};
static inline size_t planes_elems(int64_t rows, int cols) { return (size_t)((rows + 127) / 128) * ((size_t)((cols + 31) / 32) * 12288 + 2048); }
static inline Planes make_planes(u16* base, int cols, float scale = PL_SW, const float* dscale = nullptr) {
    return Planes{base, (cols + 31) / 32, scale, MI_PLANES_FP16 ? dscale : nullptr};
}

template <int MI_UNUSED = 0>
static __global__ void split_planes_kernel(const float* __restrict__ src, int ld_src, int rows, int cols, Planes dst, int row0 = 0) {
    const int cp = dst.KT * 16;
    int64_t idx = (int64_t)blockIdx.x * blockDim.x + threadIdx.x;
    const int64_t rows_pad = (int64_t)(row0 + rows + 127) / 128 * 128 - row0;
    if (idx >= rows_pad * cp) return;
    int r = (int)(idx / cp), c = (int)(idx % cp) * 2;
    float x = (r < rows && c < cols) ? src[(size_t)r * ld_src + c] : 0.f;
    float y = (r < rows && c + 1 < cols) ? src[(size_t)r * ld_src + c + 1] : 0.f;
    unsigned p[3];
    pl_split_pair(x, y, dst.s(), p);
#pragma unroll
    for (int k = 0; k < NPL; ++k) *reinterpret_cast<unsigned*>(dst.base + dst.elem(row0 + r, c, k)) = p[k];
}

__device__ __forceinline__ __amdgpu_buffer_rsrc_t uniform_rsrc(const void* p, int bytes) {
    const uint64_t a = (uint64_t)p;
    const uint32_t lo = __builtin_amdgcn_readfirstlane((uint32_t)a), hi = __builtin_amdgcn_readfirstlane((uint32_t)(a >> 32));
    return __builtin_amdgcn_make_buffer_rsrc((void*)(((uint64_t)hi << 32) | lo), 0, __builtin_amdgcn_readfirstlane(bytes), 0x00020000);
}

__device__ __forceinline__ u32x4 rsrc_words(const void* p, int bytes) {
    const uint64_t a = (uint64_t)p;
    return u32x4{(unsigned)__builtin_amdgcn_readfirstlane((uint32_t)a), (unsigned)__builtin_amdgcn_readfirstlane((uint32_t)(a >> 32)) & 0xffffu,
                 (unsigned)__builtin_amdgcn_readfirstlane(bytes), 0x00020000u};
}

struct PlanesEpilogue {
    GemmEpilogue ep;
    float out_scale = 1.f;
    const float* a_dinv = nullptr;
    unsigned* absmax = nullptr;
    int absmax_mask = 0;
    __device__ __forceinline__ float oscale() const { return a_dinv ? out_scale * a_dinv[0] : out_scale; }
    float* C = nullptr;
    int ldc = 0;
    Planes Cp;
    Planes res_pl;
    const float* residual2 = nullptr;
    int ld_res2 = 0;
    Planes res2_pl;
    float out_scale2 = 1.f;
    const int* res2_rows = nullptr;
    const float* post_mul = nullptr;
    int ld_post_mul = 0;
    __host__ __device__ bool extended() const { return res_pl.base || residual2 || res2_pl.base || post_mul; }
    float* seg_part = nullptr;
    const int* seg_src = nullptr;
    const int* seg_rowptr = nullptr;
    int seg_nodes = 0;
    const int* pair_i = nullptr;
    const int* pair_j = nullptr;
    const int* pair_e1 = nullptr;
    const int* pair_e2 = nullptr;
    const int* pair_graph = nullptr;
    const unsigned* sc_pq = nullptr;
    const unsigned* sc_gmax = nullptr;
    const float* sc_wb = nullptr;
    float* sc_dsc = nullptr;
    float* sc_dsc2 = nullptr;
    bool pair_wide = true;
    const float* diag_C0 = nullptr;
    const int* diag_node2graph = nullptr;
    const int* diag_e = nullptr;
    int diag_nodes = 0;
    int diag_block0 = 0;
    const int* m_dev = nullptr;
    int m_hint = 0;
    __device__ __forceinline__ int rows(int M) const {
        if (!m_dev) return M;
        const int md = __builtin_amdgcn_readfirstlane(*m_dev);
        return md < M ? md : M;
    }
};

__device__ __forceinline__ void act_scales_eval(float mpq, float mg, const float* __restrict__ wb, float (&dsc)[6]) {
    float bound[3];
    bound[0] = wb[0] + 2.f * mpq + mg;
    bound[1] = wb[2] + wb[1] * bound[0];
    bound[2] = wb[4] + wb[3] * bound[1] + mpq;
#pragma unroll
    for (int c = 0; c < 3; ++c) {
        float bnd = bound[c];
        int e = 14 - (int)ceilf(log2f(fmaxf(bnd, 1e-30f)));
        if (!(bnd == bnd) || bnd > 3e38f) e = -100;
        e = e > 14 ? 14 : (e < -100 ? -100 : e);
        dsc[2 * c] = exp2f((float)e);
        dsc[2 * c + 1] = exp2f(-(float)e);
    }
}

template <int TM, int TN>
__device__ __forceinline__ void planes_epilogue(const PlanesEpilogue& pe, f32x16 (&acc)[TM][TN], int row_w, int col_w, int M, int N, int l31,
                                                int kg) {
    const GemmEpilogue& ep = pe.ep;
    const float os = pe.oscale(), cps = pe.Cp.base ? pe.Cp.s() : 1.f;
    int h_srcv[TM], h_rpv[TM], h_nvalid[TM];
#pragma unroll
    for (int i = 0; i < TM; ++i) {
        h_srcv[i] = h_rpv[i] = h_nvalid[i] = 0;
        if (pe.seg_part) {
            const int rb = row_w + i * 32;
            h_nvalid[i] = M - rb < 32 ? (M - rb > 0 ? M - rb : 0) : 32;
            int r = rb + (l31 < h_nvalid[i] ? l31 : h_nvalid[i] - 1);
            r = r < M ? r : M - 1;
            r = r > 0 ? r : 0;
            h_srcv[i] = pe.seg_src[r];
        }
    }
#pragma unroll
    for (int i = 0; i < TM; ++i)
        if (pe.seg_part) h_rpv[i] = pe.seg_rowptr[h_srcv[i]];
#pragma unroll
    for (int i = 0; i < TM; ++i) {
        const int rb = row_w + i * 32;
        uint32_t starts = 0;
        const int srcv = h_srcv[i], rpv = h_rpv[i], nvalid = h_nvalid[i];
        if (pe.seg_part) {
            const int prev = __shfl_up(srcv, 1, 64);
            starts = (uint32_t)__ballot(kg == 0 && l31 < nvalid && (l31 == 0 || srcv != prev));
        }
#pragma unroll
        for (int j = 0; j < TN; ++j) {
            const int col = col_w + j * 32 + l31;
            const bool col_ok = col < N;
            const float bcol = (ep.bias && col_ok) ? ep.bias[col] : 0.f;
            float val[16];
#pragma unroll
            for (int r = 0; r < 16; ++r) {
                const int row = rb + (r & 3) + 8 * (r >> 2) + 4 * kg;
                float v = 0.f;
                if (row < M && col_ok) {
                    v = apply_epilogue<true>(ep, acc[i][j][r] * os + bcol, row, col);
                    if (pe.C) pe.C[(size_t)row * pe.ldc + col] = v;
                    if (pe.Cp.base) {
                        u16 p0, p1, p2;
                        pl_split(v, cps, p0, p1, p2);
                        pe.Cp.base[pe.Cp.elem(row, col, 0)] = p0;
                        pe.Cp.base[pe.Cp.elem(row, col, 1)] = p1;
                        if (NPL > 2) pe.Cp.base[pe.Cp.elem(row, col, 2)] = p2;
                    }
                }
                val[r] = v;
            }
            if (pe.seg_part) {
                uint32_t rem = starts;
                while (rem) {
                    const int sg = __builtin_ctz(rem);
                    rem &= rem - 1;
                    const int end = rem ? __builtin_ctz(rem) : nvalid;
                    const int node = __builtin_amdgcn_readlane(srcv, sg), rp = __builtin_amdgcn_readlane(rpv, sg);
                    const unsigned lo = (unsigned)(sg - 4 * kg), span = (unsigned)(end - sg);
                    float sum = 0.f;
#pragma unroll
                    for (int r = 0; r < 16; ++r) {
                        const unsigned c = (unsigned)((r & 3) + 8 * (r >> 2));
                        sum += (c - lo < span) ? val[r] : 0.f;
                    }
                    sum += __shfl_xor(sum, 32, 64);
                    if (kg == 0 && col_ok) {
                        const int slot = (rb >> 5) - (rp >> 5);
                        pe.seg_part[((size_t)slot * pe.seg_nodes + node) * N + col] = sum;
                    }
                }
            }
        }
    }
}

__device__ __forceinline__ void pl_add8(float (&dst)[8], const Planes& P, int row, int col) {
    const float inv = P.dscale ? P.dscale[1] : 1.f / P.scale;
    float acc[8] = {0.f, 0.f, 0.f, 0.f, 0.f, 0.f, 0.f, 0.f};
#pragma unroll
    for (int pl = NPL - 1; pl >= 0; --pl) {
        const u32x4 w = *reinterpret_cast<const u32x4*>(P.base + P.elem(row, col, pl));
#pragma unroll
        for (int k = 0; k < 4; ++k) {
            const unsigned wk = w[k];
#if MI_PLANES_FP16
            const f16x2 h = __builtin_bit_cast(f16x2, wk);
            acc[2 * k] += (float)h[0];
            acc[2 * k + 1] += (float)h[1];
#else
            acc[2 * k] += __uint_as_float(wk << 16);
            acc[2 * k + 1] += __uint_as_float(wk & 0xFFFF0000u);
#endif
        }
    }
#pragma unroll
    for (int k = 0; k < 8; ++k) dst[k] += acc[k] * inv;
}

template <int TM, int TN, bool EXT = false>
__device__ __forceinline__ void planes_epilogue_rows(const PlanesEpilogue& pe, f32x16 (&acc)[TM][TN], int row_w, int col_w, int M, int N,
                                                     int lane, float* stage) {
    const GemmEpilogue& ep = pe.ep;
    const float os = pe.oscale(), cps = pe.Cp.base ? pe.Cp.s() : 1.f;
    const int l31 = lane & 31, kg = lane >> 5;
    float amax = 0.f;
    unsigned sat = 0;
    if (pe.C && !pe.Cp.base && !ep.bias && !ep.row_bias && !ep.pre_add && !ep.pre_act && ep.act == ACT_NONE && !ep.residual && ep.out_scale == 1.f && !pe.extended()) {
#pragma unroll
        for (int i = 0; i < TM; ++i)
#pragma unroll
            for (int j = 0; j < TN; ++j) {
                const int rb = row_w + i * 32, cb = col_w + j * 32;
#pragma unroll
                for (int r = 0; r < 16; ++r) stage[((r & 3) + 8 * (r >> 2) + 4 * kg) * 36 + l31] = acc[i][j][r] * os;
                __builtin_amdgcn_wave_barrier();
#pragma unroll
                for (int it = 0; it < 4; ++it) {
                    const int rl = it * 8 + (lane >> 3), c4 = (lane & 7) * 4;
                    const int row = rb + rl, col = cb + c4;
                    const f32x4 z = *reinterpret_cast<const f32x4*>(stage + rl * 36 + c4);
                    if (row < M && col < N) {
                        amax = fmaxf(fmaxf(amax, fmaxf(fabsf(z[0]), fabsf(z[1]))), fmaxf(fabsf(z[2]), fabsf(z[3])));
                        *reinterpret_cast<f32x4*>(pe.C + (size_t)row * pe.ldc + col) = z;
                    }
                }
                __builtin_amdgcn_wave_barrier();
            }
        if (pe.absmax) {
#pragma unroll
            for (int o = 32; o > 0; o >>= 1) amax = fmaxf(amax, __shfl_xor(amax, o, 64));
            if (lane == 0) atomicMax(pe.absmax + (blockIdx.x & pe.absmax_mask), __float_as_uint(amax));
        }
        return;
    }
#pragma unroll
    for (int i = 0; i < TM; ++i)
#pragma unroll
        for (int j = 0; j < TN; ++j) {
            const int rb = row_w + i * 32, cb = col_w + j * 32;
#pragma unroll
            for (int r = 0; r < 16; ++r) stage[((r & 3) + 8 * (r >> 2) + 4 * kg) * 36 + l31] = acc[i][j][r] * os;
            __builtin_amdgcn_wave_barrier();
#pragma unroll
            for (int u = 0; u < 2; ++u) {
                const int q = lane + 64 * u, rl = q >> 2, c8 = (q & 3) * 8;
                const int row = rb + rl, col = cb + c8;
                const f32x4 z0 = *reinterpret_cast<const f32x4*>(stage + rl * 36 + c8);
                const f32x4 z1 = *reinterpret_cast<const f32x4*>(stage + rl * 36 + c8 + 4);
                if (row < M && col < N) {
                    float v[8] = {z0[0], z0[1], z0[2], z0[3], z1[0], z1[1], z1[2], z1[3]};
                    auto add8 = [&](float (&dst)[8], const float* src) {
                        const f32x4 a = *reinterpret_cast<const f32x4*>(src), b = *reinterpret_cast<const f32x4*>(src + 4);
#pragma unroll
                        for (int k = 0; k < 4; ++k) {
                            dst[k] += a[k];
                            dst[4 + k] += b[k];
                        }
                    };
                    if (ep.bias) add8(v, ep.bias + col);
                    if (ep.row_bias) {
                        float g[8] = {0.f, 0.f, 0.f, 0.f, 0.f, 0.f, 0.f, 0.f};
                        add8(g, ep.row_bias + (size_t)ep.row_group[row] * ep.ld_row_bias + col);
                        if (ep.row_bias2) add8(g, ep.row_bias2 + (size_t)ep.row_group2[row] * ep.ld_row_bias2 + col);
                        if (ep.row_bias3) add8(g, ep.row_bias3 + (size_t)ep.row_group3[row] * ep.ld_row_bias3 + col);
#pragma unroll
                        for (int k = 0; k < 8; ++k) v[k] += g[k];
                    }
                    if (ep.pre_add) add8(v, ep.pre_add + (size_t)row * ep.ld_pre_add + col);
                    if (ep.pre_act) {
                        float* d = ep.pre_act + (size_t)row * ep.ld_pre + col;
                        *reinterpret_cast<f32x4*>(d) = f32x4{v[0], v[1], v[2], v[3]};
                        *reinterpret_cast<f32x4*>(d + 4) = f32x4{v[4], v[5], v[6], v[7]};
                    }
                    if (ep.act == ACT_SILU) {
#pragma unroll
                        for (int k = 0; k < 8; ++k) v[k] = silu_fast(v[k]);
                    } else if (ep.act == ACT_SSILU) {
#pragma unroll
                        for (int k = 0; k < 8; ++k) v[k] = silu_fast(v[k]) * 1.66666666666666667f;
                    }
                    if constexpr (EXT) {
                        if (pe.post_mul) {
                            const float* src = pe.post_mul + (size_t)row * pe.ld_post_mul + col;
                            const f32x4 a = *reinterpret_cast<const f32x4*>(src), b = *reinterpret_cast<const f32x4*>(src + 4);
#pragma unroll
                            for (int k = 0; k < 4; ++k) {
                                v[k] *= a[k];
                                v[4 + k] *= b[k];
                            }
                        }
                    }
                    if (ep.residual) add8(v, ep.residual + (size_t)row * ep.ld_res + col);
                    else if constexpr (EXT) {
                        if (pe.res_pl.base) pl_add8(v, pe.res_pl, row, col);
                    }
                    if (ep.out_scale != 1.f) {
#pragma unroll
                        for (int k = 0; k < 8; ++k) v[k] *= ep.out_scale;
                    }
                    if constexpr (EXT) {
                        if (pe.residual2 || pe.res2_pl.base) {
                            if (pe.residual2) add8(v, pe.residual2 + (size_t)(pe.res2_rows ? pe.res2_rows[row] : row) * pe.ld_res2 + col);
                            else pl_add8(v, pe.res2_pl, row, col);
#pragma unroll
                            for (int k = 0; k < 8; ++k) v[k] *= pe.out_scale2;
                        }
                    }
                    if (pe.absmax) {
#pragma unroll
                        for (int k = 0; k < 8; ++k) amax = fmaxf(amax, fabsf(v[k]));
                    }
                    if (pe.C) {
                        *reinterpret_cast<f32x4*>(stage + rl * 36 + c8) = f32x4{v[0], v[1], v[2], v[3]};
                        *reinterpret_cast<f32x4*>(stage + rl * 36 + c8 + 4) = f32x4{v[4], v[5], v[6], v[7]};
                    }
                    if (pe.Cp.base) {
                        u32x4 o[3];
#pragma unroll
                        for (int k = 0; k < 4; ++k) {
                            unsigned pr[3];
                            pl_split_pair_acc(v[2 * k], v[2 * k + 1], cps, pr, sat);
                            o[0][k] = pr[0];
                            o[1][k] = pr[1];
                            o[2][k] = pr[2];
                        }
#pragma unroll
                        for (int pl = 0; pl < NPL; ++pl) *reinterpret_cast<u32x4*>(pe.Cp.base + pe.Cp.elem(row, col, pl)) = o[pl];
                    }
                }
            }
            __builtin_amdgcn_wave_barrier();
            if (pe.C) {
#pragma unroll
                for (int it = 0; it < 4; ++it) {
                    const int rl = it * 8 + (lane >> 3), c4 = (lane & 7) * 4;
                    const int row = rb + rl, col = cb + c4;
                    const f32x4 z = *reinterpret_cast<const f32x4*>(stage + rl * 36 + c4);
                    if (row < M && col < N) *reinterpret_cast<f32x4*>(pe.C + (size_t)row * pe.ldc + col) = z;
                }
                __builtin_amdgcn_wave_barrier();
            }
        }
    sat_report(sat);
    if (pe.absmax) {
#pragma unroll
        for (int o = 32; o > 0; o >>= 1) amax = fmaxf(amax, __shfl_xor(amax, o, 64));
        if (lane == 0) atomicMax(pe.absmax + (blockIdx.x & pe.absmax_mask), __float_as_uint(amax));
    }
}
template <int TM, int TN>
__device__ __forceinline__ void planes_epilogue_lean(const PlanesEpilogue& pe, f32x16 (&acc)[TM][TN], int tile, int col_w, int M, int lane) {
#if MI_PLANES_FP16
    const GemmEpilogue& ep = pe.ep;
    const int l31 = lane & 31, kg = lane >> 5;
    const float os = pe.oscale(), cps = pe.Cp.s();
    const bool has_res = pe.res_pl.base != nullptr, has_res2 = pe.res2_pl.base != nullptr, has_pm = pe.post_mul != nullptr;
    const bool has_g = ep.row_bias != nullptr, has_g2 = ep.row_bias2 != nullptr, has_rf = ep.residual != nullptr, has_rf2 = pe.residual2 != nullptr;
    const float s1 = ep.out_scale, s2 = (has_res2 || has_rf2) ? pe.out_scale2 : 1.f;
    const float post = s1 * s2 * cps;
    const float ga = ep.act == ACT_SSILU ? 1.66666666666666667f : 1.f;
    const float osx = has_g ? 1.f : os;
    const float I = 1.0f / (osx * ga * post), lin = osx * post;
    const float R1 = has_res ? (pe.res_pl.dscale ? pe.res_pl.dscale[1] : 1.f / pe.res_pl.scale) * post : 0.f;
    const float R2 = has_res2 ? (pe.res2_pl.dscale ? pe.res2_pl.dscale[1] : 1.f / pe.res2_pl.scale) * (s2 * cps) : 0.f;
    float amax = 0.f;
    unsigned sat = 0;
#pragma unroll
    for (int i = 0; i < TM; ++i) {
        const int row = tile * 128 + i * 32 + l31;
        const bool row_ok = row < M;
        const unsigned loff = (unsigned)((i * 32 + l31) * 32 + kg * 16);
        int g1 = 0, g2 = 0, r2row = row;
        if (row_ok) {
            if (has_g) g1 = ep.row_group[row];
            if (has_g2) g2 = ep.row_group2[row];
// ... 831 lines not shown
    };
    Frag f0, f1;
    auto step = [&](int kt, auto has_next, auto has_next2) {
        const unsigned char* cur = smem + (kt & 1) * BUF;
        unsigned char* nxt = smem + ((kt & 1) ^ 1) * BUF;
        if constexpr (decltype(has_next)::value) store_tiles(nxt);
        if constexpr (decltype(has_next2)::value) load_tiles(kt + 2);
        read_frag(f1, cur, 1);
        mfma_terms(f0, 0, 6);
        __syncthreads();
        if constexpr (decltype(has_next)::value) read_frag(f0, nxt, 0);
        mfma_terms(f1, 0, 6);
    };
    using yes = std::integral_constant<bool, true>;
    using no = std::integral_constant<bool, false>;

    load_tiles(0);
    store_tiles(smem);
    if (KT > 1) load_tiles(1);
    __syncthreads();
    read_frag(f0, smem, 0);
    int kt = 0;
    auto advance = [&](int kend) {
        for (; kt < kend && kt + 2 < KT; ++kt) step(kt, yes(), yes());
        for (; kt < kend; ++kt) {
            if (kt + 1 < KT) step(kt, yes(), no());
            else step(kt, no(), no());
        }
    };
    if constexpr (PAIR) {
        f32x16 accS[TM][TN];
        advance(KT / 2);
#pragma unroll
        for (int i = 0; i < TM; ++i)
#pragma unroll
            for (int j = 0; j < TN; ++j) {
                accS[i][j] = acc[i][j];
#pragma unroll
                for (int r = 0; r < 16; ++r) acc[i][j][r] = 0.f;
            }
        advance(KT);
        __syncthreads();
        planes_epilogue_pairs<TM, TN, true>(pe, accS, acc, row0 + wm * TM * 32, col0 + wn * TN * 32, M, N, lane, reinterpret_cast<float*>(smem) + wave * 2304);
        return;
    } else {
        advance(KT);
    }
    if (planes_epilogue_is_rows(pe, N)) {
        __syncthreads();
        planes_epilogue_rows<TM, TN>(pe, acc, row0 + wm * TM * 32, col0 + wn * TN * 32, M, N, lane, reinterpret_cast<float*>(smem) + wave * 1152);
    } else {
        planes_epilogue<TM, TN>(pe, acc, row0 + wm * TM * 32, col0 + wn * TN * 32, M, N, l31, kg);
    }
}

template <bool XSILU, bool F16 = false>
static __global__ __launch_bounds__(256) __attribute__((amdgpu_waves_per_eu(2, 3))) void gemm_tn_split_kernel(
    const float* __restrict__ A, int lda, const float* __restrict__ X, int ldx, float* __restrict__ P, int M, int Na, int Kx, int rows_per_split,
    int gx, int gy, int nsplit, const float* __restrict__ sa = nullptr, const float* __restrict__ sx = nullptr) {
    constexpr int PLB = 128 * 64;
    __shared__ __attribute__((aligned(16))) unsigned char smem[6 * PLB];
    unsigned char* As = smem;
    unsigned char* Xs = smem + 3 * PLB;
    const int id_ = blockIdx.x, slot_ = id_ >> 3, tile_ = slot_ % (gx * gy), bz = (slot_ / (gx * gy)) * 8 + (id_ & 7);
    if (bz >= nsplit) return;
    const int bx = tile_ % gx, by = tile_ / gx;
    const int tid = threadIdx.x, lane = tid & 63, wave = tid >> 6;
    const int wm = wave >> 1, wn = wave & 1, l31 = lane & 31, kg = lane >> 5;
    const int n0 = by * 128, k0 = bx * 128;
    const int m_begin = bz * rows_per_split, m_end = min(M, m_begin + rows_per_split);
    f32x16 acc[2][2];
#pragma unroll
    for (int i = 0; i < 2; ++i)
#pragma unroll
        for (int j = 0; j < 2; ++j)
#pragma unroll
            for (int r = 0; r < 16; ++r) acc[i][j][r] = 0.f;
    const int nl = (tid & 63) * 2, mq = tid >> 6;
    const float sca = F16 ? sa[0] : 1.f, scx = F16 ? sx[0] : 1.f, sc_out = F16 ? sa[1] * sx[1] : 1.f;
    const bool a_ok = n0 + nl < Na, x_ok = k0 + nl < Kx;
    const float* pa = A + n0 + nl;
    const float* px = X + k0 + nl;
    f32x2 ra[8], rx[8];
    auto load_slab = [&](int m0) {
#pragma unroll
        for (int t = 0; t < 8; ++t) {
            const int gm = m0 + mq * 8 + t;
            ra[t] = (a_ok && gm < m_end) ? *reinterpret_cast<const f32x2*>(pa + (size_t)gm * lda) : f32x2{0.f, 0.f};
            rx[t] = (x_ok && gm < m_end) ? *reinterpret_cast<const f32x2*>(px + (size_t)gm * ldx) : f32x2{0.f, 0.f};
        }
    };
    auto store_slab = [&]() {
#pragma unroll
        for (int u = 0; u < 2; ++u) {
            u32x4 va[3], vx[3];
#pragma unroll
            for (int t2 = 0; t2 < 4; ++t2) {
                unsigned p[3], q[3];
                float x0 = rx[2 * t2][u], x1 = rx[2 * t2 + 1][u];
                if constexpr (XSILU) {
                    x0 = silu_fast(x0);
                    x1 = silu_fast(x1);
                }
                if constexpr (F16) {
                    pl_split_pair(ra[2 * t2][u], ra[2 * t2 + 1][u], sca, p);
                    pl_split_pair(x0, x1, scx, q);
                } else {
                    split3_pair(ra[2 * t2][u], ra[2 * t2 + 1][u], p);
                    split3_pair(x0, x1, q);
                }
#pragma unroll
                for (int pl = 0; pl < 3; ++pl) {
                    va[pl][t2] = p[pl];
                    vx[pl][t2] = q[pl];
                }
            }
            const int row = nl + u, off = row * 64 + ((mq ^ ((row >> 2) & 3)) * 16);
#pragma unroll
            for (int pl = 0; pl < (F16 ? 2 : 3); ++pl) {
                *reinterpret_cast<u32x4*>(As + pl * PLB + off) = va[pl];
                *reinterpret_cast<u32x4*>(Xs + pl * PLB + off) = vx[pl];
            }
        }
    };
    load_slab(m_begin);
    for (int m0 = m_begin; m0 < m_end; m0 += 32) {
        store_slab();
        __syncthreads();
        if (m0 + 32 < m_end) load_slab(m0 + 32);
#pragma unroll
        for (int s = 0; s < 2; ++s) {
            if constexpr (F16) {
#if MI_PLANES_FP16
                f16x8 a[2][2], b[2][2];
#pragma unroll
                for (int i = 0; i < 2; ++i) {
                    const int r = (wm * 2 + i) * 32 + l31, c = (2 * s + kg) ^ ((r >> 2) & 3);
#pragma unroll
                    for (int pl = 0; pl < 2; ++pl) a[i][pl] = *reinterpret_cast<const f16x8*>(As + pl * PLB + r * 64 + c * 16);
                }
#pragma unroll
                for (int j = 0; j < 2; ++j) {
                    const int r = (wn * 2 + j) * 32 + l31, c = (2 * s + kg) ^ ((r >> 2) & 3);
#pragma unroll
                    for (int pl = 0; pl < 2; ++pl) b[j][pl] = *reinterpret_cast<const f16x8*>(Xs + pl * PLB + r * 64 + c * 16);
                }
#pragma unroll
                for (int i = 0; i < 2; ++i)
#pragma unroll
                    for (int j = 0; j < 2; ++j) {
#if !MI_TF32_CLASS
                        acc[i][j] = __builtin_amdgcn_mfma_f32_32x32x16_f16(a[i][1], b[j][0], acc[i][j], 0, 0, 0);
                        acc[i][j] = __builtin_amdgcn_mfma_f32_32x32x16_f16(a[i][0], b[j][1], acc[i][j], 0, 0, 0);
#endif
                        acc[i][j] = __builtin_amdgcn_mfma_f32_32x32x16_f16(a[i][0], b[j][0], acc[i][j], 0, 0, 0);
                    }
#endif
            } else {
            bf16x8 a[2][3], b[2][3];
#pragma unroll
            for (int i = 0; i < 2; ++i) {
                const int r = (wm * 2 + i) * 32 + l31, c = (2 * s + kg) ^ ((r >> 2) & 3);
#pragma unroll
                for (int pl = 0; pl < 3; ++pl) a[i][pl] = *reinterpret_cast<const bf16x8*>(As + pl * PLB + r * 64 + c * 16);
            }
#pragma unroll
            for (int j = 0; j < 2; ++j) {
                const int r = (wn * 2 + j) * 32 + l31, c = (2 * s + kg) ^ ((r >> 2) & 3);
#pragma unroll
                for (int pl = 0; pl < 3; ++pl) b[j][pl] = *reinterpret_cast<const bf16x8*>(Xs + pl * PLB + r * 64 + c * 16);
            }
#pragma unroll
            for (int i = 0; i < 2; ++i)
#pragma unroll
                for (int j = 0; j < 2; ++j) {
                    acc[i][j] = __builtin_amdgcn_mfma_f32_32x32x16_bf16(a[i][2], b[j][0], acc[i][j], 0, 0, 0);
                    acc[i][j] = __builtin_amdgcn_mfma_f32_32x32x16_bf16(a[i][0], b[j][2], acc[i][j], 0, 0, 0);
                    acc[i][j] = __builtin_amdgcn_mfma_f32_32x32x16_bf16(a[i][1], b[j][1], acc[i][j], 0, 0, 0);
                    acc[i][j] = __builtin_amdgcn_mfma_f32_32x32x16_bf16(a[i][1], b[j][0], acc[i][j], 0, 0, 0);
                    acc[i][j] = __builtin_amdgcn_mfma_f32_32x32x16_bf16(a[i][0], b[j][1], acc[i][j], 0, 0, 0);
                    acc[i][j] = __builtin_amdgcn_mfma_f32_32x32x16_bf16(a[i][0], b[j][0], acc[i][j], 0, 0, 0);
                }
            }
        }
        __syncthreads();
    }
    const int PK = gx * 128;
    float* Pt = P + (size_t)bz * (gy * 128) * PK;
#pragma unroll
    for (int i = 0; i < 2; ++i)
#pragma unroll
        for (int j = 0; j < 2; ++j)
#pragma unroll
            for (int r = 0; r < 16; ++r) {
                const int n = n0 + wm * 64 + i * 32 + (r & 3) + 8 * (r >> 2) + 4 * kg, k = k0 + wn * 64 + j * 32 + l31;
                Pt[(size_t)n * PK + k] = F16 ? acc[i][j][r] * sc_out : acc[i][j][r];
            }
}

extern int g_tn_split_min_rows;
extern int g_tn_split;
inline bool gemm_tn_is_split(const float* A, int lda, const float* X, int ldx, int M, int Na, int Kx) {
    return g_gemm_mode != 0 && g_tn_split && M >= g_tn_split_min_rows && Na >= 128 && Kx >= 128 && ((lda | ldx | Na | Kx) & 1) == 0 &&
           ((((uintptr_t)A) | ((uintptr_t)X)) & 7) == 0;
}
#ifdef MI_GEMM_OWNER
int gemm_tn_auto(const float* A, int lda, const float* X, int ldx, float* C, int ldc, int M, int Na, int Kx, float* scratch,
                        size_t scratch_floats, hipStream_t s, bool x_silu = false, const float* sa = nullptr, const float* sx = nullptr) {
    if (gemm_tn_is_split(A, lda, X, ldx, M, Na, Kx)) {
        const int gy = cdiv(Na, 128), gx = cdiv(Kx, 128);
        int nsplit = std::max(1, std::min(cdiv(M, 256), cdiv(tn_target_tiles(), gx * gy)));
        while (nsplit > 1 && (size_t)nsplit * gy * 128 * gx * 128 > scratch_floats) --nsplit;
        MI_CHECK((size_t)nsplit * gy * 128 * gx * 128 <= scratch_floats, MI_ENOMEM, "gemm_tn scratch too small");
        const int rows = cdiv(cdiv(M, nsplit), 32) * 32;
        nsplit = cdiv(M, rows);
        const dim3 grid(gx * gy * ((nsplit + 7) / 8 * 8));
        const bool f16 = MI_PLANES_FP16 && sa && sx;
        count_mfma(M, Na, Kx, MI_TF32_CLASS ? 1 : f16 ? 3 : 6);
        if (f16 && x_silu) hipLaunchKernelGGL((gemm_tn_split_kernel<true, true>), grid, dim3(256), 0, s, A, lda, X, ldx, scratch, M, Na, Kx, rows, gx, gy, nsplit, sa, sx);
        else if (f16) hipLaunchKernelGGL((gemm_tn_split_kernel<false, true>), grid, dim3(256), 0, s, A, lda, X, ldx, scratch, M, Na, Kx, rows, gx, gy, nsplit, sa, sx);
        else if (x_silu) hipLaunchKernelGGL((gemm_tn_split_kernel<true, false>), grid, dim3(256), 0, s, A, lda, X, ldx, scratch, M, Na, Kx, rows, gx, gy, nsplit, sa, sx);
        else hipLaunchKernelGGL((gemm_tn_split_kernel<false, false>), grid, dim3(256), 0, s, A, lda, X, ldx, scratch, M, Na, Kx, rows, gx, gy, nsplit, sa, sx);
        tn_reduce(scratch, nsplit, gy * 128, gx * 128, C, ldc, Na, Kx, s);
        MI_KERNEL_CHECK();
        return MI_OK;
    }
    MI_CHECK(!x_silu, MI_EINVAL, "gemm_tn_auto: silu on the X operand needs the bf16-pipe kernel (check gemm_tn_is_split first)");
    return gemm_tn_acc(A, lda, X, ldx, C, ldc, M, Na, Kx, scratch, scratch_floats, s);
}
#else
int gemm_tn_auto(const float* A, int lda, const float* X, int ldx, float* C, int ldc, int M, int Na, int Kx, float* scratch,
                        size_t scratch_floats, hipStream_t s, bool x_silu = false, const float* sa = nullptr, const float* sx = nullptr);
#endif

int gemm_rt(const Planes& A, const u16* Wfrag, int M, int N, int K, const PlanesEpilogue& pe, bool ext, hipStream_t s);
size_t frag_elems(int N, int K);
int pack_frag_from_planes(const Planes& W, int N, int K, u16* dst, hipStream_t s);

inline bool pairs_fit_32bit(int64_t nodes, int ld_node, int64_t graphs, int ld_graph, int64_t edges, int H) {
    const int64_t lim = (int64_t)1 << 32, u24 = (int64_t)1 << 24;
    const int64_t plane_bytes = (int64_t)planes_elems(edges, H) * 2;
    return nodes < u24 && graphs < u24 && edges < u24 && (int64_t)ld_node * 4 < u24 && (int64_t)ld_graph * 4 < u24 && (int64_t)H * 4 < u24 &&
           nodes * ld_node * 4 < lim && graphs * ld_graph * 4 < lim && edges * H * 4 < lim && plane_bytes < lim && ((int64_t)((H + 31) / 32) * 12288 + 2048) * 2 < u24;
}

#ifdef MI_GEMM_OWNER
int gemm_planes(const Planes& A, const Planes& W, int M, int N, int K, const PlanesEpilogue& pe_in, hipStream_t s) {
    MI_CHECK(A.KT >= (K + 31) / 32 && W.KT == (K + 31) / 32 && (A.KT == W.KT || K % 32 == 0), MI_EINVAL, "gemm_planes: operand plane sets do not match K");
    if (M <= 0 || N <= 0) return MI_OK;
    count_mfma(M, N, K, MI_PLANES_TERMS);
    PlanesEpilogue pe = pe_in;
    pe.out_scale = 1.f / ((A.dscale ? 1.f : A.scale) * W.scale);
    pe.a_dinv = A.dscale ? A.dscale + 1 : nullptr;
    const bool pair = pe.pair_i != nullptr;
    const bool ext = pe.extended();
    MI_CHECK(!ext || (!pair && planes_epilogue_is_rows(pe, N) && (pe.ld_post_mul & 3) == 0 && (MI_PLANES_FP16 || g_planes_variant != 1)), MI_EINVAL,
             "gemm_planes: plane-set residuals / the second merge / the multiplicand exist in the row-major epilogue of the 128-row kernel only");
    MI_CHECK(!pair || (A.KT % 2 == 0 && pe.Cp.base && pe.ep.row_bias && pe.ep.row_bias2 && pe.ep.row_bias3 && (N & 7) == 0 && !pe.ep.bias), MI_EINVAL,
             "gemm_planes: pair mode needs an even k-tile count, a plane-set output, the three gathered addends and no column bias");
    const int nct = cdiv(N, 128);
    const int Ms = (pe.m_dev && pe.m_hint > 0) ? std::min(M, pe.m_hint) : M;
#if MI_PLANES_FP16
    {
        static bool dma_attr_set = false;
        if (!dma_attr_set) {
            MI_HIP(hipFuncSetAttribute((const void*)gemm_planes_dma_kernel<0, false>, hipFuncAttributeMaxDynamicSharedMemorySize, PLANES_DMA_LDS));
            MI_HIP(hipFuncSetAttribute((const void*)gemm_planes_dma_kernel<0, true>, hipFuncAttributeMaxDynamicSharedMemorySize, PLANES_DMA_LDS));
            MI_HIP(hipFuncSetAttribute((const void*)gemm_planes_dma_kernel<1, false>, hipFuncAttributeMaxDynamicSharedMemorySize, PLANES_DMA_LDS));
            MI_HIP(hipFuncSetAttribute((const void*)gemm_planes_dma_kernel<1, true>, hipFuncAttributeMaxDynamicSharedMemorySize, PLANES_DMA_LDS));
            dma_attr_set = true;
        }
    }
#endif
#if !MI_PLANES_FP16
    if (g_planes_variant == 1 && (int64_t)cdiv(M, 256) * nct >= g_planes_db_min_tiles && !(pair && g_pair_kernel == 0)) {
        static bool attr_set = false;
        if (!attr_set) {
            MI_HIP(hipFuncSetAttribute((const void*)gemm_planes_db_kernel<false>, hipFuncAttributeMaxDynamicSharedMemorySize, GEMM_DB_LDS));
            MI_HIP(hipFuncSetAttribute((const void*)gemm_planes_db_kernel<true>, hipFuncAttributeMaxDynamicSharedMemorySize, GEMM_DB_LDS));
            attr_set = true;
        }
        const dim3 grid(nct * ((cdiv(M, 256) + 7) / 8 * 8));
        if (pair) hipLaunchKernelGGL(gemm_planes_db_kernel<true>, grid, dim3(512), GEMM_DB_LDS, s, A, W, M, N, K, pe, M);
        else hipLaunchKernelGGL(gemm_planes_db_kernel<false>, grid, dim3(512), GEMM_DB_LDS, s, A, W, M, N, K, pe, M);
    } else
#endif
    if (pair) {
        int nblk = nct * ((cdiv(M, 128) + 7) / 8 * 8);
        const bool lat = nblk <= g_planes_lat_max_blocks;
        const bool dma = MI_PLANES_FP16 && (g_planes_dma == 2 || (g_planes_dma == 1 && lat));
        if (pe.diag_C0) {
            pe.diag_block0 = nblk;
            nblk += cdiv(pe.diag_nodes, 8);
        }
        if (pe.pair_wide) {
            if (dma) hipLaunchKernelGGL((gemm_planes_dma_kernel<1, true>), dim3(nblk), dim3(256), PLANES_DMA_LDS, s, A, W, M, N, K, pe, 0);
            else if (lat) hipLaunchKernelGGL((gemm_planes_lat_kernel<1, true>), dim3(nblk), dim3(256), planes_lds_bytes(1, 2), s, A, W, M, N, K, pe, 0);
            else hipLaunchKernelGGL((gemm_planes_kernel<1, 2, true>), dim3(nblk), dim3(256), planes_lds_bytes(1, 2), s, A, W, M, N, K, pe, 0);
        } else {
            if (dma) hipLaunchKernelGGL((gemm_planes_dma_kernel<1>), dim3(nblk), dim3(256), PLANES_DMA_LDS, s, A, W, M, N, K, pe, 0);
            else if (lat) hipLaunchKernelGGL((gemm_planes_lat_kernel<1>), dim3(nblk), dim3(256), planes_lds_bytes(1, 2), s, A, W, M, N, K, pe, 0);
            else hipLaunchKernelGGL((gemm_planes_kernel<1, 2>), dim3(nblk), dim3(256), planes_lds_bytes(1, 2), s, A, W, M, N, K, pe, 0);
        }
    } else if (MI_PLANES_FP16 && W.frag && g_planes_rt && (g_planes_rt > 1 || ext) && (N & 255) == 0 && (K & 63) == 0 && K >= 128 && Ms >= g_planes_rt_min_rows &&
               planes_epilogue_is_rows(pe, N)) {
        return gemm_rt(A, W.frag, M, N, K, pe, ext, s);
    } else if (MI_PLANES_FP16 && (N & 255) == 0 && g_planes_big && (g_planes_big > 1 || !ext) && Ms >= g_planes_big_min_rows && planes_epilogue_is_rows(pe, N)) {
#if MI_PLANES_FP16
        static bool attr_set = false;
        if (!attr_set) {
            MI_HIP(hipFuncSetAttribute((const void*)gemm_planes_big_kernel<false>, hipFuncAttributeMaxDynamicSharedMemorySize, GEMM_BIG_LDS));
            MI_HIP(hipFuncSetAttribute((const void*)gemm_planes_big_kernel<true>, hipFuncAttributeMaxDynamicSharedMemorySize, GEMM_BIG_LDS));
            attr_set = true;
        }
        const dim3 grid((N >> 8) * ((cdiv(M, 256) + 7) / 8 * 8));
        if (ext) hipLaunchKernelGGL(gemm_planes_big_kernel<true>, grid, dim3(512), GEMM_BIG_LDS, s, A, W, M, N, K, pe);
        else hipLaunchKernelGGL(gemm_planes_big_kernel<false>, grid, dim3(512), GEMM_BIG_LDS, s, A, W, M, N, K, pe);
#endif
    } else if (cdiv(Ms, 128) * nct < g_planes_small_tiles) {
        if (ext) hipLaunchKernelGGL((gemm_planes_kernel<0, 1, true>), dim3(nct * ((cdiv(M, 64) + 7) / 8 * 8)), dim3(256), planes_lds_bytes(0, 1), s, A, W, M, N, K, pe, 0);
        else hipLaunchKernelGGL((gemm_planes_kernel<0, 1>), dim3(nct * ((cdiv(M, 64) + 7) / 8 * 8)), dim3(256), planes_lds_bytes(0, 1), s, A, W, M, N, K, pe, 0);
    } else if (MI_PLANES_FP16 && (g_planes_dma == 2 || (g_planes_dma == 1 && nct * ((cdiv(Ms, 128) + 7) / 8 * 8) <= g_planes_lat_max_blocks) ||
                                  (g_planes_dma == 3 && nct * ((cdiv(Ms, 128) + 7) / 8 * 8) > 256))) {
        if (ext) hipLaunchKernelGGL((gemm_planes_dma_kernel<0, true>), dim3(nct * ((cdiv(M, 128) + 7) / 8 * 8)), dim3(256), PLANES_DMA_LDS, s, A, W, M, N, K, pe, 0);
        else hipLaunchKernelGGL((gemm_planes_dma_kernel<0>), dim3(nct * ((cdiv(M, 128) + 7) / 8 * 8)), dim3(256), PLANES_DMA_LDS, s, A, W, M, N, K, pe, 0);
    } else if (nct * ((cdiv(Ms, 128) + 7) / 8 * 8) <= g_planes_lat_max_blocks) {
        if (ext) hipLaunchKernelGGL((gemm_planes_lat_kernel<0, true>), dim3(nct * ((cdiv(M, 128) + 7) / 8 * 8)), dim3(256), planes_lds_bytes(0, 2), s, A, W, M, N, K, pe, 0);
        else hipLaunchKernelGGL((gemm_planes_lat_kernel<0>), dim3(nct * ((cdiv(M, 128) + 7) / 8 * 8)), dim3(256), planes_lds_bytes(0, 2), s, A, W, M, N, K, pe, 0);
    } else {
        if (ext) hipLaunchKernelGGL((gemm_planes_kernel<0, 2, true>), dim3(nct * ((cdiv(M, 128) + 7) / 8 * 8)), dim3(256), planes_lds_bytes(0, 2), s, A, W, M, N, K, pe, 0);
        else hipLaunchKernelGGL((gemm_planes_kernel<0, 2>), dim3(nct * ((cdiv(M, 128) + 7) / 8 * 8)), dim3(256), planes_lds_bytes(0, 2), s, A, W, M, N, K, pe, 0);
    }
    MI_KERNEL_CHECK();
    return MI_OK;
}
#else
int gemm_planes(const Planes& A, const Planes& W, int M, int N, int K, const PlanesEpilogue& pe_in, hipStream_t s);
#endif

}
```

Measured before the change: 53.12.

## Compute exact per-iteration vmcnt waits via compile-time peeled k-loop forms

Replaces the hand-written k-loops in the edge and rt GEMM kernels with a templated loop that peels the prologue and epilogue and derives exact s_waitcnt vmcnt counts for each iteration at compile time. The conservative vmcnt(0) drains in the tail and first iteration go away, and short-K forms (KT of 2, 4 or 6) become possible, so the rt path now accepts K >= 64. The diagonal blocks of edge gemm1 move to the front of the grid and are vectorised into f32x4 loads and stores. The cost is more template instantiations and code size, and any miscount in the derived wait values would cause races.

```diff
diff --git a/matinvent_amd/csrc/backward.hip b/matinvent_amd/csrc/backward.hip
--- a/matinvent_amd/csrc/backward.hip
+++ b/matinvent_amd/csrc/backward.hip
@@ -1547,7 +1547,7 @@
             hipLaunchKernelGGL(split_planes_kernel<>, dim3(cdiv((int64_t)((M + 127) / 128 * 128) * PA.KT * 16, 256)), dim3(256), 0, s, A, lda, M, K, PA);
             hipLaunchKernelGGL(split_planes_kernel<>, dim3(cdiv((int64_t)((N + 127) / 128 * 128) * PW.KT * 16, 256)), dim3(256), 0, s, W, ldw, N, K, PW);
         }
-        if (MI_PLANES_FP16 && (N & 255) == 0 && (K & 63) == 0 && K >= 128) {
+        if (MI_PLANES_FP16 && (N & 255) == 0 && (K & 63) == 0 && K >= 64) {
             static u16* pf = nullptr;
             static size_t nf = 0;
             if (frag_elems(N, K) > nf) { if (pf) (void)hipFree(pf); nf = frag_elems(N, K); MI_HIP(hipMalloc((void**)&pf, nf * 2)); }
diff --git a/matinvent_amd/csrc/edge_stage.hip b/matinvent_amd/csrc/edge_stage.hip
--- a/matinvent_amd/csrc/edge_stage.hip
+++ b/matinvent_amd/csrc/edge_stage.hip
@@ -4,8 +4,10 @@
 #include <cstdlib>
 #include "net.h"
 #include "gemm_split.h"
+#include "loop_waits.h"
 #define MI_LOOP_BARRIER() __builtin_amdgcn_s_barrier()
-#define MI_RING_WAIT(w) asm volatile("s_waitcnt vmcnt(20)" : "+v"((w)[0][0]), "+v"((w)[0][1]), "+v"((w)[1][0]), "+v"((w)[1][1]))
+#define MI_LOOP_STAMP(t) asm volatile("s_memtime %0\n\ts_waitcnt lgkmcnt(0)" : "=s"(t)::"memory")
+#define MI_RING_WAIT(w, n) asm volatile("s_waitcnt vmcnt(%4)" : "+v"((w)[0][0]), "+v"((w)[0][1]), "+v"((w)[1][0]), "+v"((w)[1][1]) : "n"(n))
 
 namespace mi {
 
@@ -102,6 +104,14 @@
             asm volatile("buffer_load_dwordx4 %0, %1, %2, %3 offen offset:1024" : "=v"(w[t][1]) : "v"(voffw[t]), "s"(rsw_s), "s"(soff));
         }
     };
+    auto ring_reload = [&](int ks, u32x4 (&w)[2][2]) {
+        const int soff = __builtin_amdgcn_readfirstlane(ks * 2048);
+#pragma unroll
+        for (int t = 0; t < 2; ++t) {
+            asm volatile("buffer_load_dwordx4 %0, %1, %2, %3 offen" : "+v"(w[t][0]) : "v"(voffw[t]), "s"(rsw_s), "s"(soff));
+            asm volatile("buffer_load_dwordx4 %0, %1, %2, %3 offen offset:1024" : "+v"(w[t][1]) : "v"(voffw[t]), "s"(rsw_s), "s"(soff));
+        }
+    };
 #pragma unroll
     for (int d = 0; d < D; ++d) ring_load(d, ring[d]);
 
@@ -146,28 +156,30 @@
         }
     };
     static_assert(D == 4, "two k-tiles of ring per unrolled pair of iterations");
-#pragma unroll 1
-    for (int kt = 0; kt < KT; kt += 2) {
-#pragma unroll
-        for (int h2 = 0; h2 < 2; ++h2) {
-            const int k = kt + h2;
-            if (k == 0 || k >= KT - 3) asm volatile("s_waitcnt vmcnt(0)" ::: "memory");
-            else asm volatile("s_waitcnt vmcnt(24)" ::: "memory");
-            MI_LOOP_BARRIER();
-            if (k == 0) stamp();
-            if (k + 3 < KT) dma_tile(k + 3, (k + 3) & 3);
-            f16x8 af[4][2];
-#pragma unroll
-            for (int s2 = 0; s2 < 2; ++s2) {
-                read_a(k & 3, s2, af);
-                MI_RING_WAIT(ring[2 * h2 + s2]);
-                mma(ring[2 * h2 + s2], af);
-                if (2 * k + s2 + D < KS) ring_load(2 * k + s2 + D, ring[2 * h2 + s2]);
-                __builtin_amdgcn_sched_barrier(0);
-            }
-        }
-    }
+    unsigned long long t_first = 0, t_tail = 0;
+    auto head = [&](int k, auto hw, auto dma, auto mark) {
+        if (decltype(mark)::value == LW_MARK_TAIL && a.clk) MI_LOOP_STAMP(t_tail);
+        asm volatile("s_waitcnt vmcnt(%0)" ::"n"(decltype(hw)::value) : "memory");
+        MI_LOOP_BARRIER();
+        if (decltype(mark)::value == LW_MARK_FIRST && a.clk) MI_LOOP_STAMP(t_first);
+        if (decltype(dma)::value) dma_tile(k + 3, (k + 3) & 3);
+    };
+    auto step = [&](int k, auto slot, auto rw, auto issue) {
+        constexpr int SL = decltype(slot)::value, s2 = SL & 1;
+        f16x8 af[4][2];
+        read_a(k & 3, s2, af);
+        MI_RING_WAIT(ring[SL], decltype(rw)::value);
+        mma(ring[SL], af);
+        if (decltype(issue)::value) ring_reload(2 * k + s2 + D, ring[SL]);
+        __builtin_amdgcn_sched_barrier(0);
+    };
+    lw_k_loop<4, 4, D, lw_form(KT)>(KT, head, step);
+    stamp_i = 2;
     stamp();
+    if (a.clk && tid == 0) {
+        a.clk[(size_t)(tile * 2 + half) * 8 + 1] = t_first;
+        a.clk[(size_t)(tile * 2 + half) * 8 + 6] = t_tail;
+    }
 
     if constexpr (SAVE_Z) {
         __syncthreads();
@@ -268,7 +280,7 @@
     sat_report(sat);
 }
 
-template <bool EXT, bool LEAN = false>
+template <bool EXT, bool LEAN, int FORM>
 __global__ __launch_bounds__(256) __attribute__((amdgpu_waves_per_eu(2, 2))) void gemm_rt_kernel(Planes A, const u16* __restrict__ Wf, int M, int N, int K,
                                                                                                  PlanesEpilogue pe, unsigned long long* __restrict__ clk) {
     const int KS = K >> 4, KT = K >> 5;
@@ -315,6 +327,14 @@
             asm volatile("buffer_load_dwordx4 %0, %1, %2, %3 offen offset:1024" : "=v"(w[t][1]) : "v"(voffw[t]), "s"(rsw_s), "s"(soff));
         }
     };
+    auto ring_reload = [&](int ks, u32x4 (&w)[2][2]) {
+        const int soff = __builtin_amdgcn_readfirstlane(ks * 2048);
+#pragma unroll
+        for (int t = 0; t < 2; ++t) {
+            asm volatile("buffer_load_dwordx4 %0, %1, %2, %3 offen" : "+v"(w[t][0]) : "v"(voffw[t]), "s"(rsw_s), "s"(soff));
+            asm volatile("buffer_load_dwordx4 %0, %1, %2, %3 offen offset:1024" : "+v"(w[t][1]) : "v"(voffw[t]), "s"(rsw_s), "s"(soff));
+        }
+    };
 #pragma unroll
     for (int d = 0; d < 4; ++d) ring_load(d, ring[d]);
 
@@ -355,27 +375,25 @@
                             acc[i][j] = __builtin_amdgcn_mfma_f32_32x32x16_f16(af[i][term == 0 ? 1 : 0], __builtin_bit_cast(f16x8, w[j][term == 1 ? 1 : 0]), acc[i][j], 0, 0, 0);
         }
     };
-#pragma unroll 1
-    for (int kt = 0; kt < KT; kt += 2) {
-#pragma unroll
-        for (int h2 = 0; h2 < 2; ++h2) {
-            const int k = kt + h2;
-            if (k == 0 || k >= KT - 3) asm volatile("s_waitcnt vmcnt(0)" ::: "memory");
-            else asm volatile("s_waitcnt vmcnt(24)" ::: "memory");
-            MI_LOOP_BARRIER();
-            if (k == 0) stamp();
-            if (k + 3 < KT) dma_tile(k + 3, (k + 3) & 3);
-            f16x8 af[4][2];
-#pragma unroll
-            for (int s2 = 0; s2 < 2; ++s2) {
-                read_a(k & 3, s2, af);
-                MI_RING_WAIT(ring[2 * h2 + s2]);
-                mma(ring[2 * h2 + s2], af);
-                if (2 * k + s2 + 4 < KS) ring_load(2 * k + s2 + 4, ring[2 * h2 + s2]);
-                __builtin_amdgcn_sched_barrier(0);
-            }
-        }
-    }
+    unsigned long long t_first = 0;
+    auto head = [&](int k, auto hw, auto dma, auto mark) {
+        asm volatile("s_waitcnt vmcnt(%0)" ::"n"(decltype(hw)::value) : "memory");
+        MI_LOOP_BARRIER();
+        if (decltype(mark)::value == LW_MARK_FIRST && clk) MI_LOOP_STAMP(t_first);
+        if (decltype(dma)::value) dma_tile(k + 3, (k + 3) & 3);
+    };
+    auto step = [&](int k, auto slot, auto rw, auto issue) {
+        constexpr int SL = decltype(slot)::value, s2 = SL & 1;
+        f16x8 af[4][2];
+        read_a(k & 3, s2, af);
+        MI_RING_WAIT(ring[SL], decltype(rw)::value);
+        mma(ring[SL], af);
+        if (decltype(issue)::value) ring_reload(2 * k + s2 + 4, ring[SL]);
+        __builtin_amdgcn_sched_barrier(0);
+    };
+    lw_k_loop<4, 4, 4, FORM>(KT, head, step);
+    if (clk && tid == 0) clk[(size_t)blockIdx.x * 8 + 1] = t_first;
+    stamp_i = 2;
     __syncthreads();
     stamp();
     if constexpr (LEAN) planes_epilogue_lean<4, 2>(pe, acc, tile, cb * 256 + wave * 64, M, lane);
@@ -421,7 +439,7 @@
     for (int pl = 0; pl < 2; ++pl) *reinterpret_cast<u32x4*>(dst + ((((size_t)ct * KS + ks) * 2 + pl) * 64 + kg * 32 + l31) * 8) = pk[pl];
 }
 
-template <int D, bool WIDE>
+template <int D, bool WIDE, int FORM>
 __device__ __forceinline__ void edge_gemm1_body(const Planes& A, const u16* __restrict__ Wf, int M, int N, int K, PlanesEpilogue& pe, unsigned long long* clk) {
     extern __shared__ __attribute__((aligned(16))) unsigned char smem[];
     const int tid = threadIdx.x, lane = tid & 63, wave = __builtin_amdgcn_readfirstlane(tid >> 6);
@@ -443,32 +461,76 @@
             }
         }
     };
-    eval_scales();
-    if (pe.diag_C0 && id >= pe.diag_block0) {
-        const float cps = cps_local != 0.f ? cps_local : pe.Cp.s();
-        const int n0 = (id - pe.diag_block0) * 8, n1 = n0 + 8 < pe.diag_nodes ? n0 + 8 : pe.diag_nodes;
+    if (id < pe.diag_blocks) {
+        if (id * 8 >= pe.diag_nodes) return;
+        const bool clocked = clk && tid == 0 && id < (int)gridDim.x - pe.diag_blocks;
+        if (clocked) clk[(size_t)id * 8 + 4] = __builtin_amdgcn_s_memtime();
+        const int nch = N >> 3, items = 8 * nch;
         const float* PQ = pe.ep.row_bias;
         const int ldpq = pe.ep.ld_row_bias;
-        for (int f = 2 * tid; f < N; f += 512) {
-            const float c0 = pe.diag_C0[f], c1 = pe.diag_C0[f + 1];
-            for (int i = n0; i < n1; ++i) {
-                const int e = pe.diag_e[i], g = pe.diag_node2graph[i];
-                const float* G = pe.ep.row_bias3 + (size_t)g * pe.ep.ld_row_bias3;
-                const float v0 = c0 + ((PQ[(size_t)i * ldpq + f] + PQ[(size_t)i * ldpq + N + f]) + G[f]);
-                const float v1 = c1 + ((PQ[(size_t)i * ldpq + f + 1] + PQ[(size_t)i * ldpq + N + f + 1]) + G[f + 1]);
+        for (int base = 0; base < items; base += 512) {
+            bool ok[2];
+            int col[2], e[2], g[2];
+            f32x4 pi[2][2], pj[2][2], c0[2][2], gv[2][2];
+#pragma unroll
+            for (int u = 0; u < 2; ++u) {
+                const int item = base + tid + 256 * u, itc = item < items ? item : items - 1;
+                const int node = id * 8 + itc / nch, nc = node < pe.diag_nodes ? node : pe.diag_nodes - 1;
+                ok[u] = item < items && node < pe.diag_nodes;
+                col[u] = (itc % nch) * 8;
+                e[u] = pe.diag_e[nc];
+                g[u] = pe.diag_node2graph[nc];
+                const float* pr = PQ + (size_t)nc * ldpq + col[u];
+#pragma unroll
+                for (int h = 0; h < 2; ++h) {
+                    pi[u][h] = *reinterpret_cast<const f32x4*>(pr + 4 * h);
+                    pj[u][h] = *reinterpret_cast<const f32x4*>(pr + N + 4 * h);
+                    c0[u][h] = *reinterpret_cast<const f32x4*>(pe.diag_C0 + col[u] + 4 * h);
+                }
+            }
+#pragma unroll
+            for (int u = 0; u < 2; ++u) {
+                const float* gr = pe.ep.row_bias3 + (size_t)g[u] * pe.ep.ld_row_bias3 + col[u];
+#pragma unroll
+                for (int h = 0; h < 2; ++h) gv[u][h] = *reinterpret_cast<const f32x4*>(gr + 4 * h);
+            }
+            if (base == 0) eval_scales();
+            const float cps = cps_local != 0.f ? cps_local : pe.Cp.s();
+#pragma unroll
+            for (int u = 0; u < 2; ++u) {
+                if (!ok[u]) continue;
+                f32x4 v[2];
+                u32x4 o[NPL];
+#pragma unroll
+                for (int h = 0; h < 2; ++h) {
+#pragma unroll
+                    for (int t = 0; t < 4; ++t) v[h][t] = c0[u][h][t] + ((pi[u][h][t] + pj[u][h][t]) + gv[u][h][t]);
+#pragma unroll
+                    for (int t = 0; t < 2; ++t) {
+                        unsigned p[3];
+                        pl_split_pair(silu_fast(v[h][2 * t]), silu_fast(v[h][2 * t + 1]), cps, p);
+#pragma unroll
+                        for (int k = 0; k < NPL; ++k) o[k][2 * h + t] = p[k];
+                    }
+                }
                 if (pe.ep.pre_act) {
-                    pe.ep.pre_act[(size_t)e * pe.ep.ld_pre + f] = v0;
-                    pe.ep.pre_act[(size_t)e * pe.ep.ld_pre + f + 1] = v1;
+                    float* z = pe.ep.pre_act + (size_t)e[u] * pe.ep.ld_pre + col[u];
+                    *reinterpret_cast<f32x4*>(z) = v[0];
+                    *reinterpret_cast<f32x4*>(z + 4) = v[1];
                 }
-                unsigned p[3];
-                pl_split_pair(silu_fast(v0), silu_fast(v1), cps, p);
-#pragma unroll
-                for (int k = 0; k < NPL; ++k) *reinterpret_cast<unsigned*>(pe.Cp.base + pe.Cp.elem(e, f, k)) = p[k];
+#pragma unroll
+                for (int k = 0; k < NPL; ++k) *reinterpret_cast<u32x4*>(pe.Cp.base + pe.Cp.elem(e[u], col[u], k)) = o[k];
             }
         }
+        if (clocked) {
+            asm volatile("s_waitcnt vmcnt(0)" ::: "memory");
+            clk[(size_t)id * 8 + 5] = __builtin_amdgcn_s_memtime();
+        }
         return;
     }
-    const int slot = id >> 3, qt = slot % nq, tile = (slot / nq) * 8 + (id & 7);
+    eval_scales();
+    const int pid = id - pe.diag_blocks;
+    const int slot = pid >> 3, qt = slot % nq, tile = (slot / nq) * 8 + (pid & 7);
     const int row0 = tile * 128;
     if (row0 >= M) return;
     int stamp_i = 0;
@@ -501,6 +563,11 @@
         const int soff = __builtin_amdgcn_readfirstlane(ks * 2048);
         asm volatile("buffer_load_dwordx4 %0, %1, %2, %3 offen" : "=v"(w[0][0]) : "v"(voffw[0]), "s"(rsw_s), "s"(soff));
         asm volatile("buffer_load_dwordx4 %0, %1, %2, %3 offen offset:1024" : "=v"(w[0][1]) : "v"(voffw[0]), "s"(rsw_s), "s"(soff));
+    };
+    auto ring_reload = [&](int ks, u32x4 (&w)[NJ][2]) {
+        const int soff = __builtin_amdgcn_readfirstlane(ks * 2048);
+        asm volatile("buffer_load_dwordx4 %0, %1, %2, %3 offen" : "+v"(w[0][0]) : "v"(voffw[0]), "s"(rsw_s), "s"(soff));
+        asm volatile("buffer_load_dwordx4 %0, %1, %2, %3 offen offset:1024" : "+v"(w[0][1]) : "v"(voffw[0]), "s"(rsw_s), "s"(soff));
     };
 #pragma unroll
     for (int d = 0; d < D; ++d) ring_load(d, ring[d]);
@@ -525,8 +592,8 @@
         MI_RD128(af[3][0], 3 * 2048);        MI_RD128(af[3][1], 3 * 2048 + 8192);
 #undef MI_RD128
     };
-    auto mma = [&](u32x4 (&w)[NJ][2], f16x8 (&af)[MI][2]) {
-        asm volatile("s_waitcnt vmcnt(14)" : "+v"(w[0][0]), "+v"(w[0][1]));
+    auto mma = [&](u32x4 (&w)[NJ][2], f16x8 (&af)[MI][2], auto rw) {
+        asm volatile("s_waitcnt vmcnt(%2)" : "+v"(w[0][0]), "+v"(w[0][1]) : "n"(decltype(rw)::value));
 #pragma unroll
         for (int ip = 0; ip < 2; ++ip) {
             if (ip == 0) asm volatile("s_waitcnt lgkmcnt(4)" : "+v"(af[0][0]), "+v"(af[0][1]), "+v"(af[1][0]), "+v"(af[1][1]));
@@ -540,46 +607,48 @@
     };
     static_assert(D == 4, "two k-tiles of ring per unrolled pair of iterations");
     const int khalf = KT / 2;
-#pragma unroll 1
-    for (int kt = 0; kt < KT; kt += 2) {
-#pragma unroll
-        for (int h2 = 0; h2 < 2; ++h2) {
-            const int k = kt + h2;
-            if (k == khalf) {
-#pragma unroll
-                for (int i = 0; i < MI; ++i)
-#pragma unroll
-                    for (int j = 0; j < NJ; ++j) {
-                        accS[i][j] = acc[i][j];
-#pragma unroll
-                        for (int r = 0; r < 16; ++r) acc[i][j][r] = 0.f;
-                    }
-            }
-            if (k == 0 || k >= KT - 3) asm volatile("s_waitcnt vmcnt(0)" ::: "memory");
-            else asm volatile("s_waitcnt vmcnt(16)" ::: "memory");
-            MI_LOOP_BARRIER();
-            if (k == 0) stamp();
-            if (k + 3 < KT) dma_tile(k + 3, (k + 3) & 3);
-            f16x8 af[MI][2];
-#pragma unroll
-            for (int s2 = 0; s2 < 2; ++s2) {
-                read_a(k & 3, s2, af);
-                mma(ring[2 * h2 + s2], af);
-                if (2 * k + s2 + D < KS) ring_load(2 * k + s2 + D, ring[2 * h2 + s2]);
-                __builtin_amdgcn_sched_barrier(0);
-            }
-        }
-    }
+    unsigned long long t_first = 0, t_tail = 0;
+    auto head = [&](int k, auto hw, auto dma, auto mark) {
+        if (k == khalf) {
+#pragma unroll
+            for (int i = 0; i < MI; ++i)
+#pragma unroll
+                for (int j = 0; j < NJ; ++j) {
+                    accS[i][j] = acc[i][j];
+#pragma unroll
+                    for (int r = 0; r < 16; ++r) acc[i][j][r] = 0.f;
+                }
+        }
+        if (decltype(mark)::value == LW_MARK_TAIL && clk) MI_LOOP_STAMP(t_tail);
+        asm volatile("s_waitcnt vmcnt(%0)" ::"n"(decltype(hw)::value) : "memory");
+        MI_LOOP_BARRIER();
+        if (decltype(mark)::value == LW_MARK_FIRST && clk) MI_LOOP_STAMP(t_first);
+        if (decltype(dma)::value) dma_tile(k + 3, (k + 3) & 3);
+    };
+    auto step = [&](int k, auto slot, auto rw, auto issue) {
+        constexpr int SL = decltype(slot)::value, s2 = SL & 1;
+        f16x8 af[MI][2];
+        read_a(k & 3, s2, af);
+        mma(ring[SL], af, rw);
+        if (decltype(issue)::value) ring_reload(2 * k + s2 + D, ring[SL]);
+        __builtin_amdgcn_sched_barrier(0);
+    };
+    lw_k_loop<4, 2 * NJ, D, FORM>(KT, head, step);
+    stamp_i = 2;
     stamp();
+    if (clk && tid == 0) {
+        clk[(size_t)(tile * nq + qt) * 8 + 1] = t_first;
+        clk[(size_t)(tile * nq + qt) * 8 + 6] = t_tail;
+    }
     __syncthreads();
     planes_epilogue_pairs<MI, NJ, WIDE>(pe, accS, acc, row0 + wm * MI * 32, qt * WGC + wn * 32 * NJ, M, N, lane, reinterpret_cast<float*>(smem) + wave * 2304, cps_local);
     stamp();
 }
 
-template <int D, bool WIDE = true>
+template <int D, bool WIDE, int FORM>
 __global__ __launch_bounds__(256) __attribute__((amdgpu_waves_per_eu(2, 2))) void edge_gemm1b_kernel(Planes A, const u16* __restrict__ Wf, int M, int N, int K,
                                                                                                      PlanesEpilogue pe, unsigned long long* clk) {
-    edge_gemm1_body<D, WIDE>(A, Wf, M, N, K, pe, clk);
+    edge_gemm1_body<D, WIDE, FORM>(A, Wf, M, N, K, pe, clk);
 }
 
 unsigned long long* g_edge1_clk = nullptr;
@@ -592,8 +661,15 @@
     static std::once_flag once;
     static hipError_t attr_err = hipSuccess;
     std::call_once(once, [] {
-        attr_err = hipFuncSetAttribute((const void*)edge_gemm1b_kernel<4>, hipFuncAttributeMaxDynamicSharedMemorySize, EG2B_LDS);
-        if (attr_err == hipSuccess) attr_err = hipFuncSetAttribute((const void*)edge_gemm1b_kernel<4, false>, hipFuncAttributeMaxDynamicSharedMemorySize, EG2B_LDS);
+        auto set = [](auto form) {
+            constexpr int F = decltype(form)::value;
+            if (attr_err == hipSuccess) attr_err = hipFuncSetAttribute((const void*)edge_gemm1b_kernel<4, true, F>, hipFuncAttributeMaxDynamicSharedMemorySize, EG2B_LDS);
+            if (attr_err == hipSuccess) attr_err = hipFuncSetAttribute((const void*)edge_gemm1b_kernel<4, false, F>, hipFuncAttributeMaxDynamicSharedMemorySize, EG2B_LDS);
+        };
+        set(LwInt<0>{});
+        set(LwInt<2>{});
+        set(LwInt<4>{});
+        set(LwInt<6>{});
     });
     MI_HIP(attr_err);
     const int H = net->H, K = 2 * net->Kh;
@@ -601,12 +677,16 @@
     pe.out_scale = 1.f / (A.scale * PL_SW);
     int nblk = (H / 128) * ((cdiv(M, 128) + 7) / 8 * 8);
     if (pe.diag_C0) {
-        pe.diag_block0 = nblk;
-        nblk += cdiv(pe.diag_nodes, 8);
+        pe.diag_blocks = (cdiv(pe.diag_nodes, 8) + 7) / 8 * 8;
+        nblk += pe.diag_blocks;
     }
     const u16* Wf = net->Wffc + (size_t)layer * ((size_t)H * K * 2);
-    if (pe.pair_wide) hipLaunchKernelGGL((edge_gemm1b_kernel<4>), dim3(nblk), dim3(256), EG2B_LDS, s, A, Wf, M, H, K, pe, g_edge1_clk);
-    else hipLaunchKernelGGL((edge_gemm1b_kernel<4, false>), dim3(nblk), dim3(256), EG2B_LDS, s, A, Wf, M, H, K, pe, g_edge1_clk);
+    lw_dispatch_form(K / 32, [&](auto form) {
+        constexpr int F = decltype(form)::value;
+        if (pe.pair_wide) hipLaunchKernelGGL((edge_gemm1b_kernel<4, true, F>), dim3(nblk), dim3(256), EG2B_LDS, s, A, Wf, M, H, K, pe, g_edge1_clk);
+        else hipLaunchKernelGGL((edge_gemm1b_kernel<4, false, F>), dim3(nblk), dim3(256), EG2B_LDS, s, A, Wf, M, H, K, pe, g_edge1_clk);
+        return 0;
+    });
     MI_KERNEL_CHECK();
     return MI_OK;
 }
@@ -682,13 +762,20 @@
     static std::once_flag once;
     static hipError_t attr_err = hipSuccess;
     std::call_once(once, [] {
-        attr_err = hipFuncSetAttribute((const void*)gemm_rt_kernel<false>, hipFuncAttributeMaxDynamicSharedMemorySize, EG2B_NST * EG2B_STAGE);
-        if (attr_err == hipSuccess) attr_err = hipFuncSetAttribute((const void*)gemm_rt_kernel<true>, hipFuncAttributeMaxDynamicSharedMemorySize, EG2B_NST * EG2B_STAGE);
-        if (attr_err == hipSuccess) attr_err = hipFuncSetAttribute((const void*)gemm_rt_kernel<false, true>, hipFuncAttributeMaxDynamicSharedMemorySize, EG2B_NST * EG2B_STAGE);
+        auto set = [](auto form) {
+            constexpr int F = decltype(form)::value;
+            if (attr_err == hipSuccess) attr_err = hipFuncSetAttribute((const void*)gemm_rt_kernel<false, false, F>, hipFuncAttributeMaxDynamicSharedMemorySize, EG2B_NST * EG2B_STAGE);
+            if (attr_err == hipSuccess) attr_err = hipFuncSetAttribute((const void*)gemm_rt_kernel<true, false, F>, hipFuncAttributeMaxDynamicSharedMemorySize, EG2B_NST * EG2B_STAGE);
+            if (attr_err == hipSuccess) attr_err = hipFuncSetAttribute((const void*)gemm_rt_kernel<false, true, F>, hipFuncAttributeMaxDynamicSharedMemorySize, EG2B_NST * EG2B_STAGE);
+        };
+        set(LwInt<0>{});
+        set(LwInt<2>{});
+        set(LwInt<4>{});
+        set(LwInt<6>{});
         if (const char* e = getenv("MI_RT_LEAN")) g_rt_lean = atoi(e) & 3;
     });
     MI_HIP(attr_err);
-    MI_CHECK(Wfrag && (N & 255) == 0 && (K & 63) == 0 && K >= 128 && A.KT >= K / 32, MI_EINVAL, "gemm_rt: N % 256, K % 64, K >= 128 and a fragment-order W operand");
+    MI_CHECK(Wfrag && (N & 255) == 0 && (K & 63) == 0 && K >= 64 && A.KT >= K / 32, MI_EINVAL, "gemm_rt: N % 256, K % 64, K >= 64 and a fragment-order W operand");
     if (M <= 0) return MI_OK;
     count_mfma(M, N, K, MI_PLANES_TERMS);
     const dim3 grid((N >> 8) * ((cdiv(M, 128) + 7) / 8 * 8));
@@ -706,9 +793,13 @@
             if (g_rt_clk_ext >= 0) g_rt_clk = nullptr;
         }
     }
-    if (g_rt_lean && planes_epilogue_is_lean(pe)) hipLaunchKernelGGL((gemm_rt_kernel<false, true>), grid, dim3(256), EG2B_NST * EG2B_STAGE, s, A, Wfrag, M, N, K, pe, clk);
-    else if (ext) hipLaunchKernelGGL(gemm_rt_kernel<true>, grid, dim3(256), EG2B_NST * EG2B_STAGE, s, A, Wfrag, M, N, K, pe, clk);
-    else hipLaunchKernelGGL(gemm_rt_kernel<false>, grid, dim3(256), EG2B_NST * EG2B_STAGE, s, A, Wfrag, M, N, K, pe, clk);
+    lw_dispatch_form(K / 32, [&](auto form) {
+        constexpr int F = decltype(form)::value;
+        if (g_rt_lean && planes_epilogue_is_lean(pe)) hipLaunchKernelGGL((gemm_rt_kernel<false, true, F>), grid, dim3(256), EG2B_NST * EG2B_STAGE, s, A, Wfrag, M, N, K, pe, clk);
+        else if (ext) hipLaunchKernelGGL((gemm_rt_kernel<true, false, F>), grid, dim3(256), EG2B_NST * EG2B_STAGE, s, A, Wfrag, M, N, K, pe, clk);
+        else hipLaunchKernelGGL((gemm_rt_kernel<false, false, F>), grid, dim3(256), EG2B_NST * EG2B_STAGE, s, A, Wfrag, M, N, K, pe, clk);
+        return 0;
+    });
     MI_KERNEL_CHECK();
     return MI_OK;
 }
diff --git a/matinvent_amd/csrc/gemm_split.h b/matinvent_amd/csrc/gemm_split.h
--- a/matinvent_amd/csrc/gemm_split.h
+++ b/matinvent_amd/csrc/gemm_split.h
@@ -470,6 +470,7 @@
     const int* diag_e = nullptr;
     int diag_nodes = 0;
     int diag_block0 = 0;
+    int diag_blocks = 0;
     const int* m_dev = nullptr;
     int m_hint = 0;
     __device__ __forceinline__ int rows(int M) const {
@@ -1907,7 +1908,7 @@
             else if (lat) hipLaunchKernelGGL((gemm_planes_lat_kernel<1>), dim3(nblk), dim3(256), planes_lds_bytes(1, 2), s, A, W, M, N, K, pe, 0);
             else hipLaunchKernelGGL((gemm_planes_kernel<1, 2>), dim3(nblk), dim3(256), planes_lds_bytes(1, 2), s, A, W, M, N, K, pe, 0);
         }
-    } else if (MI_PLANES_FP16 && W.frag && g_planes_rt && (g_planes_rt > 1 || ext) && (N & 255) == 0 && (K & 63) == 0 && K >= 128 && Ms >= g_planes_rt_min_rows &&
+    } else if (MI_PLANES_FP16 && W.frag && g_planes_rt && (g_planes_rt > 1 || ext) && (N & 255) == 0 && (K & 63) == 0 && K >= 64 && Ms >= g_planes_rt_min_rows &&
                planes_epilogue_is_rows(pe, N)) {
         return gemm_rt(A, W.frag, M, N, K, pe, ext, s);
     } else if (MI_PLANES_FP16 && (N & 255) == 0 && g_planes_big && (g_planes_big > 1 || !ext) && Ms >= g_planes_big_min_rows && planes_epilogue_is_rows(pe, N)) {
diff --git a/matinvent_amd/csrc/loop_waits.h b/matinvent_amd/csrc/loop_waits.h
--- /dev/null
+++ b/matinvent_amd/csrc/loop_waits.h
@@ -0,0 +1,89 @@
+#pragma once
+
+#if defined(__HIPCC__) || defined(__CUDACC__)
+#define MI_LW_HD __host__ __device__
+#else
+#define MI_LW_HD
+#endif
+
+namespace mi {
+
+constexpr int LW_VMCNT_MAX = 63;
+constexpr int LW_CANON_KT = 12;
+
+MI_LW_HD constexpr bool lw_dma_issued(int KT, int k) { return k + 3 < KT; }
+MI_LW_HD constexpr bool lw_ring_issued(int D, int KT, int s) { return s + D < 2 * KT; }
+
+MI_LW_HD constexpr int lw_issued_at_head(int P, int R, int D, int KT, int k) {
+    int n = 3 * P + D * R;
+    for (int j = 0; j < k; ++j) n += (lw_dma_issued(KT, j) ? P : 0) + (lw_ring_issued(D, KT, 2 * j) ? R : 0) + (lw_ring_issued(D, KT, 2 * j + 1) ? R : 0);
+    return n;
+}
+MI_LW_HD constexpr int lw_issued_at_ring(int P, int R, int D, int KT, int s) {
+    const int k = s >> 1;
+    return lw_issued_at_head(P, R, D, KT, k) + (lw_dma_issued(KT, k) ? P : 0) + ((s & 1) && lw_ring_issued(D, KT, 2 * k) ? R : 0);
+}
+MI_LW_HD constexpr int lw_clamp(int n) { return n < 0 ? 0 : n > LW_VMCNT_MAX ? LW_VMCNT_MAX : n; }
+
+MI_LW_HD constexpr int lw_head_wait(int P, int R, int D, int KT, int k) {
+    const int through = k < 3 ? (k + 1) * P : lw_issued_at_head(P, R, D, KT, k - 3) + P;
+    return lw_clamp(lw_issued_at_head(P, R, D, KT, k) - through);
+}
+MI_LW_HD constexpr int lw_ring_wait(int P, int R, int D, int KT, int s) {
+    const int through = s < D ? 3 * P + (s + 1) * R : lw_issued_at_ring(P, R, D, KT, s - D) + R;
+    return lw_clamp(lw_issued_at_ring(P, R, D, KT, s) - through);
+}
+
+MI_LW_HD constexpr int lw_canon_kt(int KT) { return KT >= 8 ? LW_CANON_KT : KT; }
+MI_LW_HD constexpr int lw_canon_k(int KT, int k) { return KT < 8 ? k : k < 4 ? k : k >= KT - 4 ? k - KT + LW_CANON_KT : 4 + (k & 1); }
+
+template <int V>
+struct LwInt {
+    static constexpr int value = V;
+};
+constexpr int lw_form(int KT) { return KT >= 8 ? 0 : KT; }
+template <class F>
+inline auto lw_dispatch_form(int KT, F&& f) {
+    switch (lw_form(KT)) {
+        case 0: return f(LwInt<0>{});
+        case 6: return f(LwInt<6>{});
+        case 4: return f(LwInt<4>{});
+        default: return f(LwInt<2>{});
+    }
+}
+
+#if defined(__HIPCC__)
+constexpr int LW_MARK_FIRST = 1, LW_MARK_TAIL = 2;
+template <int P, int R, int D, int KTC, int KC, class Head, class Step>
+__device__ __forceinline__ void lw_iter(int k, Head& head, Step& step) {
+    head(k, LwInt<lw_head_wait(P, R, D, KTC, KC)>{}, LwInt<lw_dma_issued(KTC, KC)>{}, LwInt<(KC == 0 ? LW_MARK_FIRST : KC == KTC - 3 ? LW_MARK_TAIL : 0)>{});
+    step(k, LwInt<2 * (KC & 1)>{}, LwInt<lw_ring_wait(P, R, D, KTC, 2 * KC)>{}, LwInt<lw_ring_issued(D, KTC, 2 * KC)>{});
+    step(k, LwInt<2 * (KC & 1) + 1>{}, LwInt<lw_ring_wait(P, R, D, KTC, 2 * KC + 1)>{}, LwInt<lw_ring_issued(D, KTC, 2 * KC + 1)>{});
+}
+template <int P, int R, int D, int KTC, int KC, class Head, class Step>
+__device__ __forceinline__ void lw_pair(int kt, Head& head, Step& step) {
+    lw_iter<P, R, D, KTC, KC>(kt, head, step);
+    lw_iter<P, R, D, KTC, KC + 1>(kt + 1, head, step);
+}
+
+template <int P, int R, int D, int FORM, class Head, class Step>
+__device__ __forceinline__ void lw_k_loop(int KT, Head& head, Step& step) {
+    static_assert(D == 4, "two k-tiles of ring per pair of iterations");
+    static_assert(FORM == 0 || FORM == 2 || FORM == 4 || FORM == 6, "the general form or one of the short ones");
+    static_assert(lw_canon_k(8, 3) == 3 && lw_canon_k(8, 4) == 8 && lw_canon_k(10, 4) == 4 && lw_canon_k(10, 5) == 5 && lw_canon_k(10, 6) == 8, "canonical iterations");
+    if constexpr (FORM == 0) {
+        lw_pair<P, R, D, LW_CANON_KT, 0>(0, head, step);
+        lw_pair<P, R, D, LW_CANON_KT, 2>(2, head, step);
+#pragma unroll 1
+        for (int kt = 4; kt < KT - 4; kt += 2) lw_pair<P, R, D, LW_CANON_KT, 4>(kt, head, step);
+        lw_pair<P, R, D, LW_CANON_KT, 8>(KT - 4, head, step);
+        lw_pair<P, R, D, LW_CANON_KT, 10>(KT - 2, head, step);
+    } else {
+        lw_pair<P, R, D, FORM, 0>(0, head, step);
+        if constexpr (FORM >= 4) lw_pair<P, R, D, FORM, 2>(2, head, step);
+        if constexpr (FORM >= 6) lw_pair<P, R, D, FORM, 4>(4, head, step);
+    }
+}
+#endif
+
+}
```

Result: faster. 54.52, median of 6 (+2.6%).
